# swapUniba/Deep_CBRS_Amar_Renaissance

Measured on AMD Instinct MI355X. Metric: (user,item) pairs scored/sec, ML-1M basic-gnn 2-layer, 1/2/4/8 MI355X, higher is better.
Workload: dtype f32; 1 GPU; ml1m(s=64) user-item graph: N=590592 nodes, nnz(A_hat)=55909934, 12089292 test pairs; econfigs/basic-gnn.yaml grid1 BasicGCN d=8 L=2 concat, dense [24,24], clf [48,48]; one propagation + per-entity towers + all pairs (shuffled order) per step (hoisted); scale=64, parallelism=single GPU (step replayed from a hipGraph)

## Files before the change

### deep_cbrs_amar_renaissance_amd/capi.py

```python
import ctypes
import os

import torch

_HERE = os.path.dirname(os.path.abspath(__file__))
LIB_PATH = os.path.join(_HERE, 'libamar_hip.so')

ACT_NONE, ACT_RELU, ACT_SIGMOID = 0, 1, 2
ACT_CODES = {None: ACT_NONE, 'linear': ACT_NONE, 'relu': ACT_RELU, 'sigmoid': ACT_SIGMOID}
AGG_SUM, AGG_MAX, AGG_MIN = 0, 1, 2
AGG_CODES = {'sum': AGG_SUM, 'max': AGG_MAX, 'min': AGG_MIN}
SPMM_BIAS, SPMM_RELU, SPMM_ACCUM, SPMM_ACCUM_DIV, SPMM_SCALE_NEXT, SPMM_SAGE_TAIL, SPMM_LT_NOPAIRS = 1, 2, 4, 8, 16, 32, 64

_P = ctypes.c_void_p
_I32, _I64, _U32, _F32 = ctypes.c_int32, ctypes.c_int64, ctypes.c_uint32, ctypes.c_float

SIGNATURES = {
    'amar_version': (ctypes.c_int, []),
    'amar_error_string': (ctypes.c_char_p, [ctypes.c_int]),
    'amar_last_hip_error': (ctypes.c_int, []),
    'amar_spmm_csr_f32': (ctypes.c_int, [_P, _P, _P, _P, _I64, _P, _I64, _I32, _I32, _U32, _P,
                                         _P, _I64, _P, _I64, _F32, _P]),
    'amar_spmm_sj_f32': (ctypes.c_int, [_P, _P, _P, _I32, _P, _I64, _P, _I64, _I32, _I32, _U32, _P,
                                        _P, _I64, _P, _I64, _F32, _P, _I32, _P, _I64, _P]),
    'amar_spmm_xs_f32': (ctypes.c_int, [_P, _P, _P, _P, _P, _I32, _P, _I64, _I32, _P, _P, _P, _I64, _I32, _I32, _U32, _P,
                                        _P, _I64, _P, _I64, _F32, _P, _I32, _P, _I64, _P]),
    'amar_gat_lt_f32': (ctypes.c_int, [_P, _P, _P, _P, _P, _P, _P, _I32, _I32, _I32, _I32, _P, _P, _P, _P, _I64, _I32, _P, _P, _P, _P, _P, _I64,
                                       _I32, _I32, _I32, _I32, _P]),
    'amar_gat_lt_rows_per_wave': (ctypes.c_int, [_I32]),
    'amar_colmax_f32': (ctypes.c_int, [_P, _I64, _P, _P]),
    'amar_spmm_lt_f32': (ctypes.c_int, [_P, _P, _P, _P, _P, _P, _P, _I32, _I32, _I32, _P, _P, _P, _I64, _I32, _P, _P, _I64, _I32, _I32, _U32, _P,
                                        _P, _I64, _P, _I64, _F32, _P, _I32, _P, _I64, _P]),
    'amar_gat_xs_f32': (ctypes.c_int, [_P, _P, _I32, _P, _I64, _I32, _P, _P, _P, _P, _P, _P, _I64, _I32, _I32, _I32, _I32, _P]),
    'amar_gcn_layer_f32': (ctypes.c_int, [_P, _P, _P, _P, _I64, _I32, _P, _P, _I64, _P, _I32, _P, _I64, _I32, _P]),
    'amar_rowwise_xw_f32': (ctypes.c_int, [_P, _I64, _I32, _P, _I32, _P, _I64, _P, _I64, _P, _P, _P, _P, _P, _I32, _P]),
    'amar_rowwise_xw_gather_f32': (ctypes.c_int, [_P, _I64, _I32, _P, _P, _I32, _P, _I64, _P, _I32, _P]),
    'amar_sage_layer_f32': (ctypes.c_int, [_P, _P, _P, _I64, _I32, _P, _P, _I32, _P, _I64, _I32, _I32, _P]),
    'amar_sage_tail_f32': (ctypes.c_int, [_P, _I64, _P, _I64, _I32, _P, _P, _I32, _P, _I64, _I64, _P]),
    'amar_sage_layer_agg_f32': (ctypes.c_int, [_P, _P, _P, _I64, _I32, _P, _P, _I32, _P, _I64, _I32, _I32, _I32, _P]),
    'amar_sage_aggregate_f32': (ctypes.c_int, [_P, _P, _P, _I64, _I32, _P, _I64, _P, _I64, _I32, _I32, _I32, _P]),
    'amar_sage_aggregate_bwd_f32': (ctypes.c_int, [_P, _P, _P, _I64, _P, _I64, _P, _I64, _P, _I64, _I32, _P, _P, _I64, _I32, _I32, _P]),
    'amar_gat_layer_f32': (ctypes.c_int, [_P, _P, _P, _I64, _I32, _P, _P, _P, _P, _I64, _I32, _I32, _P]),
    'amar_rowwise_xw_heads_f32': (ctypes.c_int, [_P, _I64, _I32, _P, _I32, _I32, _P, _I64, _P, _P, _P, _I32, _P]),
    'amar_gat_heads_f32': (ctypes.c_int, [_P, _P, _P, _I64, _I32, _I32, _P, _P, _P, _I64, _P, _I32, _I32, _I32, _P]),
    'amar_dense_f32': (ctypes.c_int, [_P, _I64, _P, _P, _P, _P, _I64, _I64, _I32, _I32, _I32, _P]),
    'amar_dense_split_bytes': (ctypes.c_int64, [_I32, _I32]),
    'amar_dense_split_pack_f32': (ctypes.c_int, [_P, _I32, _I32, _P]),
    'amar_dense_split_f32': (ctypes.c_int, [_P, _I64, _P, _P, _P, _P, _I64, _I64, _I32, _I32, _I32, _P]),
    'amar_chain_pack_floats': (ctypes.c_int64, [_P, _I32]),
    'amar_chain_pack_f32': (ctypes.c_int, [_P, _P, _P, _I32, _P]),
    'amar_chain_f32': (ctypes.c_int, [_P, _I64, _I32, _P, _I32, _P, _I64, _I32, _P, _I32, _I32, _I32, _P, _P, _P, _I32, _P, _I64, _I64, _P]),
    'amar_chain_indexed_f32': (ctypes.c_int, [_P, _I64, _I32, _P, _I32, _P, _I64, _I32, _P, _I32, _I32, _I32, _P, _P, _P, _I32, _P, _I64, _P, _I64, _P]),
    'amar_chain_segments_f32': (ctypes.c_int, [_P, _P, _P, _I32, _P, _I32, _P, _P, _P, _I32, _P, _I64, _I64, _P]),
    'amar_chain_route': (ctypes.c_int, [_P, _I64, _I32, _P, _I32, _P, _I64, _I32, _P, _I32, _I32, _I32, _P, _P, _P, _I32, _P, _I64, _P, _I64, _P]),
    'amar_chain_segments_route': (ctypes.c_int, [_P, _P, _P, _I32, _P, _I32, _P, _P, _P, _I32, _P, _I64, _I64, _P]),
    'amar_dual_chain_f32': (ctypes.c_int, [_P, _P, _P, _P, _P, _P, _P, _P, _I32, _I32, _I32, _P, _P, _P, _I32, _P, _P, _I64, _I64, _P]),
    'amar_dual_chain_indexed_f32': (ctypes.c_int, [_P, _P, _P, _P, _P, _P, _P, _P, _I32, _I32, _I32, _P, _P, _P, _I32, _P, _P, _I64, _P, _I64, _P]),
    'amar_copy_columns_f32': (ctypes.c_int, [_P, _I64, _P, _I32, _P, _I64, _I64, _I32, _P]),
    'amar_scatter_f32': (ctypes.c_int, [_P, _P, _P, _I64, _I64, _P, _I32, _P]),
    'amar_reduce_layers_f32': (ctypes.c_int, [_P, _I64, _I32, _I32, _P, _I64, _I64, _I32, _P]),
    'amar_reduce_layers_wsum_f32': (ctypes.c_int, [_P, _I64, _I32, _I32, _P, _P, _I64, _I64, _P]),
    'amar_reduce_layers_wsum_bwd_scratch': (ctypes.c_int64, []),
    'amar_reduce_layers_wsum_bwd_f32': (ctypes.c_int, [_P, _I64, _I32, _I32, _P, _P, _I64, _P, _I64, _P, _P, _I64, _P]),
    'amar_act_bwd_f32': (ctypes.c_int, [_P, _I64, _P, _I64, _P, _I64, _I64, _I32, _I32, _P]),
    'amar_wgrad_scratch_floats': (ctypes.c_int64, [_I64, _I32, _I32]),
    'amar_wgrad_f32': (ctypes.c_int, [_P, _I64, _P, _I64, _I64, _I32, _I32, _P, _P, _P, _P]),
    'amar_dense_stack_f32': (ctypes.c_int, [_P, _I64, _P, _P, _I64, _I32, _P, _P, _P, _P, _P, _P, _I64, _P]),
    'amar_dense_stack_pair_f32': (ctypes.c_int, [_P, _P, _P]),
    'amar_dense_stack_route': (ctypes.c_int, [_P, _I64, _P, _P, _I64, _I32, _P, _P, _P, _P, _P, _P, _I64, _P]),
    'amar_dense_stack_bwd_groups': (ctypes.c_int64, [_I64]),
    'amar_dense_stack_bwd_workspace_floats': (ctypes.c_int64, [_I64, _I32, _P]),
    'amar_dense_stack_bwd_pair_f32': (ctypes.c_int, [_P, _P, _P]),
    'amar_dense_stack_bwd_f32': (ctypes.c_int, [_P, _I64, _P, _I64, _I32, _P, _P, _P, _P, _P, _P, _I64, _P, _P, _P, _I32, _I64, _P]),
    'amar_dense_stack_bwd_route': (ctypes.c_int, [_P, _I64, _P, _I64, _I32, _P, _P, _P, _P, _P, _P, _I64, _P, _P, _P, _I32, _I64, _P]),
    'amar_dense_bwd_workspace_floats': (ctypes.c_int64, [_I64, _I32, _I32]),
    'amar_dense_bwd_groups': (ctypes.c_int64, [_I64]),
    'amar_dense_bwd_f32': (ctypes.c_int, [_P, _I64, _P, _I64, _P, _I64, _P, _I32, _P, _I64, _P, _P, _P, _I64, _P, _I64, _I32, _I32, _P]),
    'amar_dense_bwd_route': (ctypes.c_int, [_P, _I64, _P, _I64, _P, _I64, _P, _I32, _P, _I64, _P, _P, _P, _I64, _I64, _I32, _I32, _P]),
    'amar_bce_grad_f32': (ctypes.c_int, [_P, _I64, _P, _P, _P, _I64, _P]),
    'amar_wgrad_route': (ctypes.c_int, [_P, _I64, _P, _I64, _I64, _I32, _I32, _P, _P, _P]),
    'amar_scatter_add_rows_route': (ctypes.c_int, [_I64, _I32, _P]),
    'amar_scatter_add_rows_f32': (ctypes.c_int, [_P, _I64, _P, _I32, _P, _I64, _I64, _I32, _P]),
    'amar_add_inplace_f32': (ctypes.c_int, [_P, _I64, _P, _I64, _I64, _I32, _F32, _P]),
    'amar_row_affine_f32': (ctypes.c_int, [_P, _I64, _P, _I64, _P, _P, _I64, _I64, _I32, _P]),
    'amar_l2norm_fwd_f32': (ctypes.c_int, [_P, _I64, _P, _I64, _P, _P, _I64, _I64, _I32, _I32, _P]),
    'amar_l2norm_bwd_f32': (ctypes.c_int, [_P, _I64, _P, _I64, _P, _P, _I64, _I64, _I32, _I32, _P]),
    'amar_gat_bwd_f32': (ctypes.c_int, [_P, _P, _P, _I64, _I32, _P, _P, _P, _I64, _P, _I64, _P, _P, _P, _P, _P, _P, _P, _P, _I64,
                                        _I32, _I32, _P]),
    'amar_gat_bwd_directed_f32': (ctypes.c_int, [_P, _P, _P, _P, _P, _I64, _I32, _P, _P, _P, _I64, _P, _I64, _P, _P, _P, _P, _P, _P, _P, _P, _I64,
                                                 _I32, _I32, _P]),
    'amar_gat_heads_bwd_f32': (ctypes.c_int, [_P, _P, _P, _P, _P, _I64, _I32, _I32, _P, _P, _I64, _P, _I64, _P, _P, _P, _P, _P, _P, _P, _P, _I64,
                                              _I32, _I32, _I32, _P]),
    'amar_attention_mix_f32': (ctypes.c_int, [_P, _I64, _P, _I64, _P, _I64, _P, _I64, _P, _I64, _I64, _I32, _P]),
    'amar_attention_mix_bwd_f32': (ctypes.c_int, [_P, _I64, _P, _I64, _P, _I64, _P, _I64, _P, _I64, _P, _P, _P, _P, _I64, _I32, _P]),
    'amar_add3_act_f32': (ctypes.c_int, [_P, _I64, _P, _I64, _P, _I64, _P, _I64, _I64, _I32, _I32, _P]),
    'amar_locality_scale_f32': (ctypes.c_int, [_P, _I64, _P, _P, _I64, _I64, _I32, _P]),
    'amar_locality_scale_bwd_f32': (ctypes.c_int, [_P, _I64, _P, _I64, _P, _P, _I64, _P, _I64, _I32, _I32, _P]),
    'amar_transpose_f32': (ctypes.c_int, [_P, _I32, _I32, _P, _P]),
    'amar_adam_f32': (ctypes.c_int, [_P, _P, _P, _P, _I64, _F32, _F32, _F32, _F32, _F32, _P]),
    'amar_adam_advance_f32': (ctypes.c_int, [_P, _F32, _F32, _F32, _P]),
    'amar_adam_dev_f32': (ctypes.c_int, [_P, _P, _P, _P, _I64, _P, _F32, _F32, _F32, _F32, _P]),
    'amar_optim_state_arrays': (ctypes.c_int, [_I32, _I32, _F32]),
    'amar_optim_advance_f32': (ctypes.c_int, [_P, _I32, _I32, _P, _P]),
    'amar_optim_f32': (ctypes.c_int, [_I32, _I32, _P, _P, _P, _P, _P, _P, _I64, _P, _F32, _P]),
    'amar_optim_multi_f32': (ctypes.c_int, [_I32, _I32, _P, _P, _I32, _I64, _P, _F32, _P, _P]),
    'amar_grad_clip_workspace_floats': (ctypes.c_int64, [_I32, _I64]),
    'amar_grad_clip_f32': (ctypes.c_int, [_I32, _F32, _P, _I32, _I64, _P, _P, _F32, _P, _P]),
    'amar_bpr_grad_f32': (ctypes.c_int, [_P, _I64, _P, _P, _I64, _P]),
    'amar_bpr_sample_i32': (ctypes.c_int, [_P, _P, _P, _P, _I32, ctypes.c_uint64, _P, _I32, _I32, _P, _P, _P, _P]),
    'amar_loss_counters': (ctypes.c_int32, []),
    'amar_loss_grad_f32': (ctypes.c_int, [_I32, _P, _P, _I64, _P, _P, _P, _I64, _P, _P]),
    'amar_dropout_f32': (ctypes.c_int, [_P, _I64, _P, _I64, _I64, _I32, ctypes.c_uint64, _P, _U32, _U32, _F32, _P]),
    'amar_dropout_advance': (ctypes.c_int, [_P, _P]),
    'amar_gat_layer_dropout_f32': (ctypes.c_int, [_P, _P, _P, _I64, _I32, _P, _P, _P, _P, _I64, _I32, _I32,
                                                  ctypes.c_uint64, _P, _U32, _U32, _F32, _P]),
    'amar_gat_bwd_dropout_f32': (ctypes.c_int, [_P, _P, _P, _I64, _I32, _P, _P, _P, _I64, _P, _I64, _P, _P, _P, _P, _P, _P, _P, _P, _I64,
                                                _I32, _I32, ctypes.c_uint64, _P, _U32, _U32, _F32, _P]),
    'amar_gat_bwd_directed_dropout_f32': (ctypes.c_int, [_P, _P, _P, _P, _P, _I64, _I32, _P, _P, _P, _I64, _P, _I64, _P, _P, _P, _P, _P, _P, _P, _P,
                                                         _I64, _I32, _I32, ctypes.c_uint64, _P, _U32, _U32, _F32, _P]),
    'amar_csr_transpose_i32': (ctypes.c_int, [_P, _P, _I32, _I32, _I32, _P, _P, _P, _P, _P]),
    'amar_adam_multi_f32': (ctypes.c_int, [_P, _I32, _I64, _P, _F32, _F32, _F32, _F32, _P, _P]),
    'amar_sum_into_f32': (ctypes.c_int, [_P, _I64, _F32, _P, _P]),
    'amar_topk_segmented_f32': (ctypes.c_int, [_P, _P, _P, _I32, _I32, _P, _P, _P]),
    'amar_recommend_slices': (ctypes.c_int32, [_I64, _I32, _P, _I32, _I32]),
    'amar_recommend_f32': (ctypes.c_int, [_P, _I64, _I32, _P, _I64, _I32, _I32, _P, _P, _P, _I32, _I32, _P, _I64, _P, _P,
                                          _I32, _I32, _P, _P, _P, _P, _P]),
}

_lib = None


class AmarError(RuntimeError):
    pass


def load():
    global _lib
    if _lib is None:
        if not os.path.exists(LIB_PATH):
            raise AmarError(
                "{} is missing: build it with `python -c 'import __graft_entry__ as g; g.build()'` "
                "or `make -C deep_cbrs_amar_renaissance_amd/csrc`. The HIP path has no fallback.".format(LIB_PATH))
# ... 565 lines not shown

class ConcatTable:

    def __init__(self, tables):
        tables = list(tables)
        if not tables:
            raise ValueError("ConcatTable: at least one table expected")
        rows = int(tables[0].shape[0])
        if any(t.dim() != 2 or int(t.shape[0]) != rows or t.dtype != torch.float32 for t in tables):
            raise ValueError("ConcatTable: float32 [rows, w] tables with equal row counts expected")
        self.in_place = all(int(t.shape[1]) % 4 == 0 for t in tables)
        self.segments = tables
        self.shape = (rows, sum(int(t.shape[1]) for t in tables))
        self.device, self.dtype = tables[0].device, torch.float32

    def __getitem__(self, key):
        if not isinstance(key, slice) or key.step not in (None, 1):
            raise TypeError("ConcatTable supports contiguous row slices only")
        return ConcatTable([t[key] for t in self.segments])

    def materialize(self):
        out = torch.empty(self.shape, dtype=torch.float32, device=self.device)
        off = 0
        for t in self.segments:
            copy_columns(t, out[:, off:off + t.shape[1]])
            off += t.shape[1]
        return out


def _chain_segments_args(table, wpack, dims, acts, out, ids=None, base=0):
    P = out.shape[0]
    segs = table.segments
    if ids is not None and ids.numel() != P:
        raise ValueError("chain: ids must have one id per output row")
    if ids is None and table.shape[0] < P:
        raise ValueError("chain: input blocks have fewer rows than the output")
    n = len(segs)
    ptrs = (ctypes.c_void_p * n)(*[_ptr(t, torch.float32, 'segment') for t in segs])
    lds = (ctypes.c_int64 * n)(*[_ld(t, 'segment') for t in segs])
    ws = (ctypes.c_int32 * n)(*[int(t.shape[1]) for t in segs])
    dims_c = (ctypes.c_int32 * len(dims))(*dims)
    acts_c = (ctypes.c_int32 * len(acts))(*[ACT_CODES[a] for a in acts])
    return [ptrs, lds, ws, n, _ptr(ids, torch.int32, 'ids'), int(base), _ptr(wpack, torch.float32, 'wpack'), dims_c, acts_c, len(acts),
            _ptr(out, torch.float32, 'out'), _ld(out, 'out'), P]


def chain_segments(table, wpack, dims, acts, out, ids=None, base=0):
    code = load().amar_chain_segments_f32(*_chain_segments_args(table, wpack, dims, acts, out, ids=ids, base=base), _stream())
    if code == -2:
        return False
    _check(code, 'amar_chain_segments_f32')
    return True


def _chain_args(A, wpack, dims, acts, out, ids_a=None, base_a=0, B=None, ids_b=None, base_b=0, sum_inputs=False, in_act=None, out_index=None):
    P = out.shape[0]
    Da, Db = A.shape[1], (B.shape[1] if B is not None else 0)
    for ids, nm in ((ids_a, 'ids_a'), (ids_b, 'ids_b')):
        if ids is not None and ids.numel() != P:
            raise ValueError("chain: {} must have one id per output row".format(nm))
    if ids_a is None and A.shape[0] < P or (B is not None and ids_b is None and B.shape[0] < P):
        raise ValueError("chain: input blocks have fewer rows than the output")
    dims_c = (ctypes.c_int32 * len(dims))(*dims)
    acts_c = (ctypes.c_int32 * len(acts))(*[ACT_CODES[a] for a in acts])
    if out_index is not None and out_index.numel() != P:
        raise ValueError("chain: out_index must have one entry per output row")
    return [_ptr(A, torch.float32, 'A'), _ld(A, 'A'), Da, _ptr(ids_a, torch.int32, 'ids_a'), int(base_a),
            _ptr(B, torch.float32, 'B'), _ld(B, 'B') if B is not None else 0, Db, _ptr(ids_b, torch.int32, 'ids_b'), int(base_b),
            1 if sum_inputs else 0, ACT_CODES[in_act],
            _ptr(wpack, torch.float32, 'wpack'), dims_c, acts_c, len(acts),
            _ptr(out, torch.float32, 'out'), _ld(out, 'out'), _ptr(out_index, torch.int32, 'out_index'), P]


def chain(A, wpack, dims, acts, out, ids_a=None, base_a=0, B=None, ids_b=None, base_b=0, sum_inputs=False, in_act=None, out_index=None):
    if isinstance(A, ConcatTable):
        if A.in_place and B is None and not sum_inputs and out_index is None and chain_segments(A, wpack, dims, acts, out, ids=ids_a, base=base_a):
            return
        A = A.materialize()
    args = _chain_args(A, wpack, dims, acts, out, ids_a=ids_a, base_a=base_a, B=B, ids_b=ids_b, base_b=base_b, sum_inputs=sum_inputs,
                       in_act=in_act, out_index=out_index)
    _check(load().amar_chain_indexed_f32(*args, _stream()), 'amar_chain_indexed_f32' if out_index is not None else 'amar_chain_f32')


CHAIN_KERNEL_GENERIC, CHAIN_KERNEL_PIPE, CHAIN_KERNEL_ROWS = 0, 1, 2


class ChainRouteInfo(ctypes.Structure):
    _fields_ = [(name, ctypes.c_int32) for name in ('kernel', 'maxt', 'full', 'am', 'split', 'scatter', 'shape', 'lastlin', 'seg', 'has_dot',
                                                    'layers', 'threads')] + [('blocks', ctypes.c_int64), ('lds_bytes', ctypes.c_int64)]

    def as_dict(self):
        d = {name: int(getattr(self, name)) for name, _ in self._fields_}
        for name in ('full', 'split', 'scatter', 'lastlin', 'seg', 'has_dot'):
            d[name] = bool(d[name])
        return d


def chain_shape(*tiles):
    code = len(tiles) - 1
    for j, t in enumerate(tiles):
        code |= t << (3 * (j + 1))
    return code


def chain_route(A, wpack, dims, acts, out, ids_a=None, base_a=0, B=None, ids_b=None, base_b=0, sum_inputs=False, in_act=None, out_index=None):
    info = ChainRouteInfo()
    if isinstance(A, ConcatTable):
        if not (A.in_place and B is None and not sum_inputs and out_index is None):
            raise ValueError("chain_route: this ConcatTable call is assembled first; ask about the assembled table")
        args = _chain_segments_args(A, wpack, dims, acts, out, ids=ids_a, base=base_a)
        _check(load().amar_chain_segments_route(*args, ctypes.byref(info)), 'amar_chain_segments_route')
        return info.as_dict()
    args = _chain_args(A, wpack, dims, acts, out, ids_a=ids_a, base_a=base_a, B=B, ids_b=ids_b, base_b=base_b, sum_inputs=sum_inputs,
                       in_act=in_act, out_index=out_index)
    _check(load().amar_chain_route(*args, ctypes.byref(info)), 'amar_chain_route')
    return info.as_dict()


def dual_chain_supported(D, n_branch_dims_equal, trunk_dims):
    return (D % 16 == 0 and D <= 64 and n_branch_dims_equal and len(trunk_dims) >= 3 and trunk_dims[0] == 2 * D
            and trunk_dims[-1] == 1 and len(set(trunk_dims[1:-1])) == 1 and trunk_dims[1] <= 64 and trunk_dims[1] % 4 == 0)


def dual_chain(tables_a, tables_b, ids_a, ids_b, bases_a, bases_b, D, in_act, branch_acts, trunk_dims, trunk_acts, wpack, out,
               out_index=None):
    P = out.shape[0]
    arr = lambda vals, ctype: (ctype * 2)(*vals)
    A = arr([_ptr(t, torch.float32, 'A') for t in tables_a], ctypes.c_void_p)
    B = arr([_ptr(t, torch.float32, 'B') for t in tables_b], ctypes.c_void_p)
    IA = arr([_ptr(t, torch.int32, 'ida') for t in ids_a], ctypes.c_void_p)
    IB = arr([_ptr(t, torch.int32, 'idb') for t in ids_b], ctypes.c_void_p)
    for ids in list(ids_a) + list(ids_b):
        if ids is not None and ids.numel() != P:
            raise ValueError("dual_chain: one id per output row expected")
    lda = arr([_ld(t, 'A') for t in tables_a], ctypes.c_int64)
    ldb = arr([_ld(t, 'B') for t in tables_b], ctypes.c_int64)
    ba, bb = arr([int(b) for b in bases_a], ctypes.c_int32), arr([int(b) for b in bases_b], ctypes.c_int32)
    bacts = (ctypes.c_int32 * max(1, len(branch_acts)))(*[ACT_CODES[a] for a in branch_acts])
    tdims = (ctypes.c_int32 * len(trunk_dims))(*trunk_dims)
    tacts = (ctypes.c_int32 * len(trunk_acts))(*[ACT_CODES[a] for a in trunk_acts])
    if out_index is not None and out_index.numel() != P:
        raise ValueError("dual_chain: out_index must have one entry per output row")
    code = load().amar_dual_chain_indexed_f32(A, lda, IA, ba, B, ldb, IB, bb, D, ACT_CODES[in_act], len(branch_acts), bacts,
                                              tdims, tacts, len(trunk_acts), _ptr(wpack, torch.float32, 'wpack'),
                                              _ptr(out, torch.float32, 'out'), _ld(out, 'out'), _ptr(out_index, torch.int32, 'out_index'),
                                              P, _stream())
    _check(code, 'amar_dual_chain_f32' if out_index is None else 'amar_dual_chain_indexed_f32')


def scatter(src, index, dst, window_off=None, n_windows=1):
    n = int(index.numel())
    if src.numel() < n or (window_off is not None and window_off.numel() != n_windows + 1):
        raise ValueError("scatter: one source value per index and n_windows + 1 window offsets expected")
    if n == 0:
        return
    _check(load().amar_scatter_f32(_ptr(src, torch.float32, 'src'), _ptr(index, torch.int32, 'index'), _ptr(dst, torch.float32, 'dst'),
                                   _ld(dst, 'dst') if dst.dim() == 2 else 1, n, _ptr(window_off, torch.int32, 'window_off'),
                                   int(n_windows), _stream()), 'amar_scatter_f32')


def copy_columns(src, dst, ids=None, base=0):
    n = ids.numel() if ids is not None else src.shape[0]
    if src.shape[1] != dst.shape[1] or dst.shape[0] != n:
        raise ValueError("copy_columns: shapes differ")
    code = load().amar_copy_columns_f32(_ptr(src, torch.float32, 'src'), _ld(src, 'src'),
                                        _ptr(ids, torch.int32, 'ids'), int(base),
                                        _ptr(dst, torch.float32, 'dst'), _ld(dst, 'dst'),
                                        n, src.shape[1], _stream())
    _check(code, 'amar_copy_columns_f32')


def reduce_layers(cat, n_layers, width, out, mean=False):
    if cat.shape[1] != n_layers * width or tuple(out.shape) != (cat.shape[0], width):
        raise ValueError("reduce_layers: cat [n, n_layers*width], out [n, width] expected")
    code = load().amar_reduce_layers_f32(_ptr(cat, torch.float32, 'cat'), _ld(cat, 'cat'), n_layers, width,
                                         _ptr(out, torch.float32, 'out'), _ld(out, 'out'), cat.shape[0],
                                         1 if mean else 0, _stream())
    _check(code, 'amar_reduce_layers_f32')


def reduce_layers_wsum(cat, n_layers, width, w, out):
    if cat.shape[1] != n_layers * width or tuple(out.shape) != (cat.shape[0], width) or w.numel() != n_layers or not w.is_contiguous():
        raise ValueError("reduce_layers_wsum: cat [n, n_layers*width], w [n_layers], out [n, width] expected")
    code = load().amar_reduce_layers_wsum_f32(_ptr(cat, torch.float32, 'cat'), _ld(cat, 'cat'), n_layers, width, _ptr(w, torch.float32, 'w'),
                                              _ptr(out, torch.float32, 'out'), _ld(out, 'out'), cat.shape[0], _stream())
    _check(code, 'amar_reduce_layers_wsum_f32')


def reduce_layers_wsum_bwd(cat, n_layers, width, w, d_out, d_cat, dw):
    n = cat.shape[0]
    if (cat.shape[1] != n_layers * width or tuple(d_cat.shape) != tuple(cat.shape) or tuple(d_out.shape) != (n, width)
            or w.numel() != n_layers or dw.numel() != n_layers or not w.is_contiguous() or not dw.is_contiguous()):
        raise ValueError("reduce_layers_wsum_bwd: cat / d_cat [n, n_layers*width], d_out [n, width], w / dw [n_layers] expected")
    scratch = torch.empty(int(load().amar_reduce_layers_wsum_bwd_scratch()), dtype=torch.float32, device=cat.device)
    code = load().amar_reduce_layers_wsum_bwd_f32(_ptr(cat, torch.float32, 'cat'), _ld(cat, 'cat'), n_layers, width, _ptr(w, torch.float32, 'w'),
                                                  _ptr(d_out, torch.float32, 'd_out'), _ld(d_out, 'd_out'),
                                                  _ptr(d_cat, torch.float32, 'd_cat'), _ld(d_cat, 'd_cat'), _ptr(dw, torch.float32, 'dw'),
                                                  _ptr(scratch, torch.float32, 'scratch'), n, _stream())
    _check(code, 'amar_reduce_layers_wsum_bwd_f32')


def adam_advance(state, learning_rate, beta_1, beta_2):
    if state.numel() != 2 or not state.is_contiguous():
        raise ValueError("adam_advance: state must be 2 contiguous floats (t, lr_t)")
    _check(load().amar_adam_advance_f32(_ptr(state, torch.float32, 'state'), float(learning_rate), float(beta_1), float(beta_2),
                                        _stream()), 'amar_adam_advance_f32')


def adam_dev(w, g, m, v, state, beta_1, beta_2, epsilon, l2=0.0):
    if not (w.is_contiguous() and g.is_contiguous() and m.is_contiguous() and v.is_contiguous()) or \
            not (w.numel() == g.numel() == m.numel() == v.numel()):
        raise ValueError("adam_dev: contiguous tensors of equal size expected")
    code = load().amar_adam_dev_f32(_ptr(w, torch.float32, 'w'), _ptr(g, torch.float32, 'g'), _ptr(m, torch.float32, 'm'),
                                    _ptr(v, torch.float32, 'v'), w.numel(), _ptr(state, torch.float32, 'state'), float(beta_1),
                                    float(beta_2), float(epsilon), float(l2), _stream())
    _check(code, 'amar_adam_dev_f32')


class DeferredGradient:

    def __init__(self, partials, groups, shape):
        self.partials, self.groups, self.shape = partials, int(groups), tuple(shape)

    def materialize(self):
        parts = self.partials.view(self.groups, -1)
        total = torch.zeros_like(parts[0])
        for g in range(self.groups):
            total += parts[g]
        return total.view(self.shape)


def flat_gradient(g):
    return g if isinstance(g, DeferredGradient) else g.contiguous().view(-1)


class AdamSlot(ctypes.Structure):
    _fields_ = [('w', ctypes.c_void_p), ('g', ctypes.c_void_p), ('m', ctypes.c_void_p), ('v', ctypes.c_void_p),
# ... 819 lines not shown
```

### deep_cbrs_amar_renaissance_amd/csrc/amar_chain.hip

```cpp
#include "amar_common.h"
#include <stdlib.h>
#include <string.h>

namespace {

typedef float f32x4 __attribute__((ext_vector_type(4)));

constexpr int CHAIN_MAX_LAYERS = 8;
constexpr int CHAIN_MAX_SEG = 8;

struct ChainArgs {
    const float *A; int64_t lda; int Da; const int32_t *ids_a; int base_a;
    int n_seg; const float *seg[CHAIN_MAX_SEG]; int64_t seg_ld[CHAIN_MAX_SEG]; int seg_off[CHAIN_MAX_SEG + 1];
    const float *B; int64_t ldb; int Db; const int32_t *ids_b; int base_b;
    const float *wpack; int wpack_floats;
    int sum_inputs, in_act;
    int n_layers;
    int kt[CHAIN_MAX_LAYERS], nt[CHAIN_MAX_LAYERS], act[CHAIN_MAX_LAYERS];
    int w_off[CHAIN_MAX_LAYERS], b_off[CHAIN_MAX_LAYERS];
    int has_dot, dot_off, dot_bias_off, dot_act, dot_kt;
    int n_out;
    float *out; int64_t ldo; int64_t P;
    const int32_t *out_index;
};

__device__ __forceinline__ int64_t chain_out_row(const ChainArgs &a, int64_t p) { return a.out_index ? (int64_t)a.out_index[p] : p; }

__device__ __forceinline__ float chain_act(float v, int act) {
    if (act == AMAR_ACT_RELU) return fmaxf(v, 0.f);
    if (act == AMAR_ACT_SIGMOID) return 1.f / (1.f + expf(-v));
    return v;
}

template <bool RELU>
__device__ __forceinline__ float chain_act_t(float v, int act) { return RELU ? fmaxf(v, 0.f) : chain_act(v, act); }

template <int MAXT, int PT, bool FULL, int AM>
__global__ __launch_bounds__(256) void chain_kernel(const ChainArgs a) {
    constexpr bool RELU = AM != 0;
    extern __shared__ __attribute__((aligned(16))) float w_lds[];
    for (int i = threadIdx.x * 4; i < a.wpack_floats; i += blockDim.x * 4)
        *reinterpret_cast<float4 *>(&w_lds[i]) = *reinterpret_cast<const float4 *>(a.wpack + i);
    __syncthreads();

    const int lane = threadIdx.x & 63, g = lane >> 4, col = lane & 15;
    const int64_t pairs_per_wave = 16 * PT;
    const int64_t wave0 = (int64_t)blockIdx.x * 4 + (threadIdx.x >> 6);
    const int64_t stride = (int64_t)gridDim.x * 4 * pairs_per_wave;

    for (int64_t base = wave0 * pairs_per_wave; base < a.P; base += stride) {
        f32x4 x[MAXT][PT];
#pragma unroll
        for (int pt = 0; pt < PT; ++pt) {
            const int64_t p = base + 16 * pt + col;
            const bool ok = p < a.P;
            const int64_t ra = ok ? (a.ids_a ? (int64_t)a.ids_a[p] - a.base_a : p) : 0;
            const int64_t rb = (ok && a.Db) ? (a.ids_b ? (int64_t)a.ids_b[p] - a.base_b : p) : 0;
#pragma unroll
            for (int t = 0; t < MAXT; ++t) {
                const int f = 16 * t + 4 * g;
                f32x4 v = {0.f, 0.f, 0.f, 0.f};
                if ((FULL || t < a.kt[0]) && ok) {
                    if (a.sum_inputs) {
                        if (f < a.Da) {
                            const f32x4 va = *reinterpret_cast<const f32x4 *>(a.A + ra * a.lda + f);
                            const f32x4 vb = *reinterpret_cast<const f32x4 *>(a.B + rb * a.ldb + f);
                            v = va + vb;
#pragma unroll
                            for (int r = 0; r < 4; ++r) v[r] = chain_act_t<RELU>(v[r], a.in_act);
                        }
                    } else if (f < a.Da) v = *reinterpret_cast<const f32x4 *>(a.A + ra * a.lda + f);
                    else if (f < a.Da + a.Db) v = *reinterpret_cast<const f32x4 *>(a.B + rb * a.ldb + (f - a.Da));
                }
                x[t][pt] = v;
            }
        }
        for (int l = 0; l < a.n_layers; ++l) {
            const int KT = FULL ? MAXT : a.kt[l], NT = FULL ? MAXT : a.nt[l];
            const float *wl = w_lds + a.w_off[l];
            const float *bl = w_lds + a.b_off[l];
            f32x4 y[MAXT][PT];
#pragma unroll
            for (int m = 0; m < MAXT; ++m) {
                if (FULL || m < NT) {
                    const f32x4 b4 = *reinterpret_cast<const f32x4 *>(bl + 16 * m + 4 * g);
#pragma unroll
                    for (int pt = 0; pt < PT; ++pt) y[m][pt] = b4;
#pragma unroll
                    for (int t = 0; t < MAXT; ++t) {
                        if (FULL || t < KT) {
                            const f32x4 w4 = *reinterpret_cast<const f32x4 *>(wl + ((m * KT + t) * 64 + lane) * 4);
#pragma unroll
                            for (int r = 0; r < 4; ++r)
#pragma unroll
                                for (int pt = 0; pt < PT; ++pt)
                                    y[m][pt] = __builtin_amdgcn_mfma_f32_16x16x4f32(w4[r], x[t][pt][r], y[m][pt], 0, 0, 0);
                        }
                    }
                }
            }
            const int act = a.act[l];
            if (AM == 2 && l == a.n_layers - 1) {
#pragma unroll
                for (int m = 0; m < MAXT; ++m)
#pragma unroll
                    for (int pt = 0; pt < PT; ++pt) {
                        const f32x4 zero = {0.f, 0.f, 0.f, 0.f};
                        x[m][pt] = (FULL || m < NT) ? y[m][pt] : zero;
                    }
            } else {
#pragma unroll
                for (int m = 0; m < MAXT; ++m)
#pragma unroll
                    for (int pt = 0; pt < PT; ++pt) {
                        f32x4 v = {0.f, 0.f, 0.f, 0.f};
                        if (FULL || m < NT) {
                            v = y[m][pt];
#pragma unroll
                            for (int r = 0; r < 4; ++r) v[r] = chain_act_t<RELU>(v[r], act);
                        }
                        x[m][pt] = v;
                    }
            }
        }
        if (a.has_dot) {
            const float *wd = w_lds + a.dot_off;
            const float bd = w_lds[a.dot_bias_off];
#pragma unroll
            for (int pt = 0; pt < PT; ++pt) {
                float s = 0.f;
#pragma unroll
                for (int t = 0; t < MAXT; ++t) {
                    if (FULL || t < a.dot_kt) {
                        const f32x4 w4 = *reinterpret_cast<const f32x4 *>(wd + 16 * t + 4 * g);
#pragma unroll
                        for (int r = 0; r < 4; ++r) s = fmaf(x[t][pt][r], w4[r], s);
                    }
                }
                s += __shfl_xor(s, 16, 64);
                s += __shfl_xor(s, 32, 64);
                const int64_t p = base + 16 * pt + col;
                if (g == 0 && p < a.P) a.out[chain_out_row(a, p) * a.ldo] = chain_act(s + bd, a.dot_act);
            }
        } else {
#pragma unroll
            for (int pt = 0; pt < PT; ++pt) {
                const int64_t p = base + 16 * pt + col;
#pragma unroll
                for (int m = 0; m < MAXT; ++m) {
                    const int f = 16 * m + 4 * g;
                    if (p < a.P && f < a.n_out) *reinterpret_cast<f32x4 *>(a.out + chain_out_row(a, p) * a.ldo + f) = x[m][pt];
                }
            }
        }
    }
}

__device__ __forceinline__ float relu_bits(float v) { return __int_as_float(max(__float_as_int(v), 0)); }

constexpr int chain_shape(int nl, int t0, int t1, int t2 = 0, int t3 = 0) { return nl | t0 << 3 | t1 << 6 | t2 << 9 | t3 << 12; }
constexpr int shape_nl(int s) { return s & 7; }
constexpr int shape_t(int s, int j) { return (s >> (3 * (j + 1))) & 7; }
constexpr int shape_maxt(int s) {
    int m = 0;
    for (int j = 0; j <= shape_nl(s); ++j) m = shape_t(s, j) > m ? shape_t(s, j) : m;
    return m;
}

template <int SHAPE, int PT, bool LASTLIN, bool SEG>
__global__ __launch_bounds__(256) void chain_rows_kernel(const ChainArgs a) {
    constexpr int NL = shape_nl(SHAPE), T0 = shape_t(SHAPE, 0), TN = shape_t(SHAPE, NL), MAXT = shape_maxt(SHAPE);
    extern __shared__ __attribute__((aligned(16))) float w_lds[];
    for (int i = threadIdx.x * 4; i < a.wpack_floats; i += blockDim.x * 4)
        *reinterpret_cast<float4 *>(&w_lds[i]) = *reinterpret_cast<const float4 *>(a.wpack + i);
    __syncthreads();

    const int lane = threadIdx.x & 63, g = lane >> 4, col = lane & 15;
    constexpr uint32_t rows_per_wave = 16 * PT;
    const uint32_t stride = gridDim.x * 4 * rows_per_wave;
    const uint32_t P = (uint32_t)a.P, last = P - 1;
    const uint32_t lda = (uint32_t)a.lda * 4u;
    const int f_last = 16 * (T0 - 1) + 4 * g;
    const bool tail_ok = f_last < a.Da;
    const char *Ag = reinterpret_cast<const char *>(a.A) + 16 * g;
    const int tail_off = tail_ok ? 64 * (T0 - 1) : -16 * g;
    const char *seg_base[SEG ? T0 : 1];
    uint32_t seg_ldb[SEG ? T0 : 1];
    if constexpr (SEG) {
#pragma unroll
        for (int t = 0; t < T0; ++t) {
            const int f = 16 * t + 4 * g;
            int sidx = 0;
            for (int j = 1; j < a.n_seg; ++j) sidx = (f < a.Da && f >= a.seg_off[j]) ? j : sidx;
            seg_base[t] = reinterpret_cast<const char *>(a.seg[sidx] + (f < a.Da ? f - a.seg_off[sidx] : 0));
            seg_ldb[t] = (uint32_t)a.seg_ld[sidx] * 4u;
        }
    }

    f32x4 xin[MAXT][PT];
    auto gather = [&](uint32_t b) {
#pragma unroll
        for (int pt = 0; pt < PT; ++pt) {
            const uint32_t p = min(b + 16 * pt + col, last);
            const uint32_t row = a.ids_a ? (uint32_t)(a.ids_a[p] - a.base_a) : p;
            const char *pa = Ag + (uint64_t)row * lda;
#pragma unroll
            for (int t = 0; t < T0; ++t) {
                if constexpr (SEG) xin[t][pt] = *reinterpret_cast<const f32x4 *>(seg_base[t] + (uint64_t)row * seg_ldb[t]);
                else xin[t][pt] = *reinterpret_cast<const f32x4 *>(pa + (t == T0 - 1 ? tail_off : 64 * t));
            }
        }
    };

    uint32_t base = (blockIdx.x * 4 + (threadIdx.x >> 6)) * rows_per_wave;
    if (base >= P) return;
    gather(base);
    for (; base < P; base += stride) {
        f32x4 x[MAXT][PT];
#pragma unroll
        for (int l = 0; l < NL; ++l) {
            const int KT = shape_t(SHAPE, l), NT = shape_t(SHAPE, l + 1);
            const float *wl = w_lds + a.w_off[l];
            const float *bl = w_lds + a.b_off[l];
            f32x4 y[MAXT][PT];
#pragma unroll
            for (int m = 0; m < MAXT; ++m) {
                if (m < NT) {
                    const f32x4 b4 = *reinterpret_cast<const f32x4 *>(bl + 16 * m + 4 * g);
#pragma unroll
                    for (int pt = 0; pt < PT; ++pt) y[m][pt] = b4;
#pragma unroll
                    for (int t = 0; t < MAXT; ++t) {
                        if (t < KT) {
                            const f32x4 w4 = *reinterpret_cast<const f32x4 *>(wl + ((m * KT + t) * 64 + lane) * 4);
#pragma unroll
                            for (int r = 0; r < 4; ++r)
#pragma unroll
                                for (int pt = 0; pt < PT; ++pt) {
                                    float xv = l == 0 ? xin[t][pt][r] : x[t][pt][r];
                                    if (l == 0 && t == T0 - 1) xv = tail_ok ? xv : 0.f;
                                    y[m][pt] = __builtin_amdgcn_mfma_f32_16x16x4f32(w4[r], xv, y[m][pt], 0, 0, 0);
                                }
                        }
                    }
                }
            }
            if (l == 0) gather(base + stride);
#pragma unroll
            for (int m = 0; m < MAXT; ++m)
#pragma unroll
                for (int pt = 0; pt < PT; ++pt)
                    if (m < NT) {
#pragma unroll
                        for (int r = 0; r < 4; ++r) x[m][pt][r] = (LASTLIN && l == NL - 1) ? y[m][pt][r] : relu_bits(y[m][pt][r]);
                    }
        }
#pragma unroll
        for (int pt = 0; pt < PT; ++pt) {
            const uint32_t p = base + 16 * pt + col;
            float *po = a.out + (int64_t)p * a.ldo + 4 * g;
#pragma unroll
            for (int m = 0; m < TN; ++m)
                if (p < P && 16 * m + 4 * g < a.n_out) *reinterpret_cast<f32x4 *>(po + 16 * m) = x[m][pt];
        }
    }
}


typedef uint32_t u32x4 __attribute__((ext_vector_type(4)));
typedef __bf16 bf16x8 __attribute__((ext_vector_type(8)));

struct Split3 { uint32_t h, m, l; };
typedef float f32x2 __attribute__((ext_vector_type(2)));
typedef uint32_t u32x2 __attribute__((ext_vector_type(2)));
__device__ __forceinline__ Split3 split_pair(float a, float b) {
    const f32x2 x = {a, b};
    const u32x2 xb = __builtin_bit_cast(u32x2, x);
    Split3 q;
    q.h = __builtin_amdgcn_perm(xb[1], xb[0], 0x07060302u);
    const f32x2 r1 = x - __builtin_bit_cast(f32x2, xb & 0xffff0000u);
    const u32x2 r1b = __builtin_bit_cast(u32x2, r1);
    q.m = __builtin_amdgcn_perm(r1b[1], r1b[0], 0x07060302u);
    const f32x2 r2 = r1 - __builtin_bit_cast(f32x2, r1b & 0xffff0000u);
    const u32x2 r2b = __builtin_bit_cast(u32x2, r2);
    q.l = __builtin_amdgcn_perm(r2b[1], r2b[0], 0x07060302u);
    return q;
}

struct Split3x4 { u32x4 h, m, l; };
__device__ __forceinline__ Split3x4 split_tiles(const f32x4 &t0, const f32x4 &t1) {
    const Split3 q0 = split_pair(t0[0], t0[1]), q1 = split_pair(t0[2], t0[3]), q2 = split_pair(t1[0], t1[1]), q3 = split_pair(t1[2], t1[3]);
    Split3x4 o;
    o.h[0] = q0.h; o.h[1] = q1.h; o.h[2] = q2.h; o.h[3] = q3.h;
    o.m[0] = q0.m; o.m[1] = q1.m; o.m[2] = q2.m; o.m[3] = q3.m;
    o.l[0] = q0.l; o.l[1] = q1.l; o.l[2] = q2.l; o.l[3] = q3.l;
    return o;
}
__device__ __forceinline__ f32x4 split_mfma(const u32x4 *w, const Split3x4 &x, f32x4 acc) {
    const bf16x8 wh = __builtin_bit_cast(bf16x8, w[0]), wm = __builtin_bit_cast(bf16x8, w[64]), wl = __builtin_bit_cast(bf16x8, w[128]);
    const bf16x8 xh = __builtin_bit_cast(bf16x8, x.h), xm = __builtin_bit_cast(bf16x8, x.m), xl = __builtin_bit_cast(bf16x8, x.l);
    acc = __builtin_amdgcn_mfma_f32_16x16x32_bf16(wl, xh, acc, 0, 0, 0);
    acc = __builtin_amdgcn_mfma_f32_16x16x32_bf16(wh, xl, acc, 0, 0, 0);
    acc = __builtin_amdgcn_mfma_f32_16x16x32_bf16(wm, xm, acc, 0, 0, 0);
    acc = __builtin_amdgcn_mfma_f32_16x16x32_bf16(wm, xh, acc, 0, 0, 0);
    acc = __builtin_amdgcn_mfma_f32_16x16x32_bf16(wh, xm, acc, 0, 0, 0);
    acc = __builtin_amdgcn_mfma_f32_16x16x32_bf16(wh, xh, acc, 0, 0, 0);
    return acc;
}

template <int MAXT, int PT, bool SCATTER, bool SPLIT>
__global__ __launch_bounds__(256) void chain_pipe_kernel(const ChainArgs a) {
    extern __shared__ __attribute__((aligned(16))) float w_lds[];
    for (int i = threadIdx.x * 4; i < a.wpack_floats; i += blockDim.x * 4)
        *reinterpret_cast<float4 *>(&w_lds[i]) = *reinterpret_cast<const float4 *>(a.wpack + i);
    __syncthreads();

    const int lane = threadIdx.x & 63, g = lane >> 4, col = lane & 15;
    constexpr int KS = (MAXT + 1) / 2;
    constexpr bool BIASK = SPLIT && (MAXT & 1);
    u32x4 *frag = reinterpret_cast<u32x4 *>(w_lds + ((a.wpack_floats + 3) & ~3));
    if (SPLIT) {
        for (int idx = threadIdx.x >> 6; idx < a.n_layers * MAXT * KS; idx += 4) {
            const int l = idx / (MAXT * KS), m = (idx % (MAXT * KS)) / KS, sk = idx % KS;
            const float *wl = w_lds + a.w_off[l];
            const f32x4 wa = *reinterpret_cast<const f32x4 *>(wl + ((m * MAXT + 2 * sk) * 64 + lane) * 4);
            f32x4 wb = {0.f, 0.f, 0.f, 0.f};
            if (2 * sk + 1 < MAXT) wb = *reinterpret_cast<const f32x4 *>(wl + ((m * MAXT + 2 * sk + 1) * 64 + lane) * 4);
            else if (BIASK && g == 0) wb[0] = w_lds[a.b_off[l] + 16 * m + col];
            u32x4 *dst = frag + idx * 3 * 64 + lane;
            const Split3 q0 = split_pair(wa[0], wa[1]), q1 = split_pair(wa[2], wa[3]), q2 = split_pair(wb[0], wb[1]), q3 = split_pair(wb[2], wb[3]);
            u32x4 h, mm, lo;
            h[0] = q0.h; h[1] = q1.h; h[2] = q2.h; h[3] = q3.h;
            mm[0] = q0.m; mm[1] = q1.m; mm[2] = q2.m; mm[3] = q3.m;
            lo[0] = q0.l; lo[1] = q1.l; lo[2] = q2.l; lo[3] = q3.l;
            dst[0] = h; dst[64] = mm; dst[128] = lo;
        }
        __syncthreads();
    }
    constexpr uint32_t pairs_per_wave = 16 * PT;
    const uint32_t wave0 = blockIdx.x * 4 + (threadIdx.x >> 6);
    const uint32_t stride = gridDim.x * 4 * pairs_per_wave;
    const uint32_t P = (uint32_t)a.P, last = P - 1;
    const char *Ag = reinterpret_cast<const char *>(a.A + 4 * g), *Bg = reinterpret_cast<const char *>(a.B + 4 * g);
// ... 707 lines not shown
            a.has_dot = 1; a.dot_off = off; a.dot_kt = tiles16(K); a.dot_act = act;
            off += 16 * tiles16(K);
            a.dot_bias_off = off;
            off += 4;
        } else {
            maxw = N > maxw ? N : maxw;
            a.kt[a.n_layers] = tiles16(K); a.nt[a.n_layers] = tiles16(N); a.act[a.n_layers] = act;
            a.w_off[a.n_layers] = off;
            off += tiles16(N) * tiles16(K) * 256;
            a.b_off[a.n_layers] = off;
            off += 16 * tiles16(N);
            a.n_layers++;
            a.n_out = N;
        }
    }
    a.wpack_floats = off;
    if (a.n_layers < 1) return AMAR_EINVAL;
    if (!a.has_dot && ((ldo & 3) || ldo < a.n_out || (a.n_out & 3) || !amar_aligned16(out))) return AMAR_EINVAL;
    if (a.has_dot && ldo < 1) return AMAR_EINVAL;
    if (maxw > 128 || (size_t)off * sizeof(float) > 150 * 1024) return AMAR_EUNSUPPORTED;
    const size_t lds_bytes = (size_t)off * sizeof(float);
    const int maxt = maxw <= 48 ? 3 : (maxw <= 64 ? 4 : 8);
    bool full = (dims[0] + 15) / 16 == maxt && (!a.has_dot || a.dot_kt == maxt);
    for (int l = 0; l < a.n_layers; ++l) full = full && a.kt[l] == maxt && a.nt[l] == maxt;
    bool relu = !a.sum_inputs || a.in_act == AMAR_ACT_RELU, relu_but_last = relu && !a.has_dot;
    for (int l = 0; l < a.n_layers; ++l) {
        relu = relu && a.act[l] == AMAR_ACT_RELU;
        relu_but_last = relu_but_last && a.act[l] == (l == a.n_layers - 1 ? AMAR_ACT_NONE : AMAR_ACT_RELU);
    }
    const int am = relu ? 1 : (relu_but_last ? 2 : 0);
    r.maxt = maxt; r.full = full; r.am = am; r.has_dot = a.has_dot; r.layers = a.n_layers; r.threads = 256;
    r.lds_bytes = (int64_t)lds_bytes;
    const int64_t tiles = (P + 4 * 16 * 2 - 1) / (4 * 16 * 2);
    const bool a_dot_ok = !a.has_dot || a.dot_kt == maxt;
    const bool small_tables = lda < (1ll << 30) && ldb < (1ll << 30) && P < (1ll << 30) - (4ll << 20);
    if (relu && a.sum_inputs && a.in_act == AMAR_ACT_RELU && full && a_dot_ok && a.ids_a && a.ids_b && a.Da == 16 * maxt &&
        a.Db == a.Da && maxt <= 4 && lds_bytes <= 64 * 1024 && small_tables && (a.has_dot || !a.out_index)) {
        static const bool f32_only = getenv("AMAR_PAIR_MFMA") && !strcmp(getenv("AMAR_PAIR_MFMA"), "f32");
        const size_t split_bytes = (((size_t)off + 3) & ~(size_t)3) * sizeof(float) + (size_t)a.n_layers * maxt * ((maxt + 1) / 2) * 3 * 1024;
        r.kernel = AMAR_CHAIN_KERNEL_PIPE;
        r.split = !f32_only && split_bytes <= 64 * 1024;
        r.scatter = a.out_index != nullptr;
        r.blocks = tiles > 1536 ? 1536 : tiles;
        if (r.split) r.lds_bytes = (int64_t)split_bytes;
        return AMAR_OK;
    }
    if ((am == 1 || am == 2) && !a.sum_inputs && a.Db == 0 && !a.has_dot && !a.out_index && a.n_layers <= 3 &&
        maxt <= 4 && lds_bytes <= 64 * 1024 && lda < (1ll << 30) && P < (1ll << 30) - (4ll << 20)) {
        const int shape = chain_shape(a.n_layers, a.kt[0], a.nt[0], a.n_layers > 1 ? a.nt[1] : 0, a.n_layers > 2 ? a.nt[2] : 0);
        if (chain_rows_shape_known(shape)) {
            r.kernel = AMAR_CHAIN_KERNEL_ROWS;
            r.shape = shape; r.lastlin = am == 2; r.seg = n_seg > 0;
            r.blocks = tiles > 1024 ? 1024 : tiles;
            return AMAR_OK;
        }
    }
    if (n_seg > 0 && P > 0) return AMAR_EUNSUPPORTED;
    r.kernel = AMAR_CHAIN_KERNEL_GENERIC;
    r.blocks = tiles > 4096 ? 4096 : tiles;
    return AMAR_OK;
}

int amar_chain_route(const float *A, int64_t lda, int32_t Da, const int32_t *ids_a, int32_t base_a,
                     const float *B, int64_t ldb, int32_t Db, const int32_t *ids_b, int32_t base_b,
                     int32_t sum_inputs, int32_t in_act,
                     const float *wpack, const int32_t *dims, const int32_t *acts, int32_t n_layers,
                     float *out, int64_t ldo, const int32_t *out_index, int64_t P, amar_chain_route_info *info) {
    if (!info) return AMAR_EINVAL;
    ChainArgs a;
    return chain_route(A, lda, Da, ids_a, base_a, B, ldb, Db, ids_b, base_b, sum_inputs, in_act, wpack, dims, acts, n_layers, out, ldo, out_index, P,
                       0, nullptr, nullptr, nullptr, a, *info);
}

int amar_chain_segments_route(const float *const *seg, const int64_t *seg_ld, const int32_t *seg_width, int32_t n_seg,
                              const int32_t *ids, int32_t base,
                              const float *wpack, const int32_t *dims, const int32_t *acts, int32_t n_layers,
                              float *out, int64_t ldo, int64_t P, amar_chain_route_info *info) {
    if (!info) return AMAR_EINVAL;
    int64_t da = 0;
    if (const int rc = chain_segments_check(seg, seg_ld, seg_width, n_seg, &da)) return rc;
    ChainArgs a;
    return chain_route(seg[0], seg_ld[0], (int32_t)da, ids, base, nullptr, 0, 0, nullptr, 0, 0, AMAR_ACT_NONE, wpack, dims, acts, n_layers, out, ldo,
                       nullptr, P, n_seg, seg, seg_ld, seg_width, a, *info);
}

static int chain_run(const float *A, int64_t lda, int32_t Da, const int32_t *ids_a, int32_t base_a,
                     const float *B, int64_t ldb, int32_t Db, const int32_t *ids_b, int32_t base_b,
                     int32_t sum_inputs, int32_t in_act,
                     const float *wpack, const int32_t *dims, const int32_t *acts, int32_t n_layers,
                     float *out, int64_t ldo, const int32_t *out_index, int64_t P, amar_stream_t stream,
                     int32_t n_seg, const float *const *seg, const int64_t *seg_ld, const int32_t *seg_width) {
    ChainArgs a;
    amar_chain_route_info r;
    if (const int rc = chain_route(A, lda, Da, ids_a, base_a, B, ldb, Db, ids_b, base_b, sum_inputs, in_act, wpack, dims, acts, n_layers, out, ldo,
                                   out_index, P, n_seg, seg, seg_ld, seg_width, a, r))
        return rc;
    if (r.blocks == 0) return AMAR_OK;
    hipStream_t st = static_cast<hipStream_t>(stream);
    const dim3 grid((unsigned)r.blocks), block((unsigned)r.threads);
    const size_t lds = (size_t)r.lds_bytes;
    if (r.kernel == AMAR_CHAIN_KERNEL_PIPE) {
#define AMAR_PIPE_LAUNCH(MT, SC)                                                                                          \
        do {                                                                                                              \
            if (r.split) hipLaunchKernelGGL((chain_pipe_kernel<MT, 2, SC, true>), grid, block, lds, st, a);               \
            else hipLaunchKernelGGL((chain_pipe_kernel<MT, 2, SC, false>), grid, block, lds, st, a);                      \
        } while (0)
        if (r.scatter) {
            if (r.maxt == 3) AMAR_PIPE_LAUNCH(3, true); else AMAR_PIPE_LAUNCH(4, true);
        } else {
            if (r.maxt == 3) AMAR_PIPE_LAUNCH(3, false); else AMAR_PIPE_LAUNCH(4, false);
        }
#undef AMAR_PIPE_LAUNCH
        return amar_check_launch();
    }
    if (r.kernel == AMAR_CHAIN_KERNEL_ROWS) {
#define AMAR_ROWS_CASE(NLL, A0, A1, A2, A3)                                                                                      \
        case chain_shape(NLL, A0, A1, A2, A3):                                                                                   \
            if (r.seg) {                                                                                                         \
                if (r.lastlin) hipLaunchKernelGGL((chain_rows_kernel<chain_shape(NLL, A0, A1, A2, A3), 2, true, true>), grid, block, lds, st, a);   \
                else hipLaunchKernelGGL((chain_rows_kernel<chain_shape(NLL, A0, A1, A2, A3), 2, false, true>), grid, block, lds, st, a);            \
            } else if (r.lastlin) hipLaunchKernelGGL((chain_rows_kernel<chain_shape(NLL, A0, A1, A2, A3), 2, true, false>), grid, block, lds, st, a);   \
            else hipLaunchKernelGGL((chain_rows_kernel<chain_shape(NLL, A0, A1, A2, A3), 2, false, false>), grid, block, lds, st, a);            \
            break;
        switch (r.shape) {
        AMAR_ROWS_SHAPES(AMAR_ROWS_CASE)
        default: return AMAR_EUNSUPPORTED;
        }
#undef AMAR_ROWS_CASE
        return amar_check_launch();
    }
#define AMAR_CHAIN_LAUNCH(MT)                                                                                           \
    do {                                                                                                                \
        auto kern = r.full ? (r.am == 1 ? chain_kernel<MT, 2, true, 1> : r.am == 2 ? chain_kernel<MT, 2, true, 2>       \
                                                                                 : chain_kernel<MT, 2, true, 0>)        \
                           : (r.am == 1 ? chain_kernel<MT, 2, false, 1> : r.am == 2 ? chain_kernel<MT, 2, false, 2>     \
                                                                                  : chain_kernel<MT, 2, false, 0>);     \
        if (lds > 64 * 1024 &&                                                                                          \
            hipFuncSetAttribute(reinterpret_cast<const void *>(kern), hipFuncAttributeMaxDynamicSharedMemorySize,       \
                                (int)lds) != hipSuccess)                                                                \
            return AMAR_ELAUNCH;                                                                                        \
        hipLaunchKernelGGL(kern, grid, block, lds, st, a);                                                              \
    } while (0)
    if (r.maxt == 3) AMAR_CHAIN_LAUNCH(3); else if (r.maxt == 4) AMAR_CHAIN_LAUNCH(4); else AMAR_CHAIN_LAUNCH(8);
#undef AMAR_CHAIN_LAUNCH
    return amar_check_launch();
}

int amar_dual_chain_f32(const float *const *A, const int64_t *lda, const int32_t *const *ida, const int32_t *base_a,
                        const float *const *B, const int64_t *ldb, const int32_t *const *idb, const int32_t *base_b,
                        int32_t D, int32_t in_act, int32_t n_branch, const int32_t *branch_acts,
                        const int32_t *trunk_dims, const int32_t *trunk_acts, int32_t n_trunk,
                        const float *wpack, float *out, int64_t ldo, int64_t P, amar_stream_t stream) {
    return amar_dual_chain_indexed_f32(A, lda, ida, base_a, B, ldb, idb, base_b, D, in_act, n_branch, branch_acts, trunk_dims, trunk_acts,
                                       n_trunk, wpack, out, ldo, nullptr, P, stream);
}

int amar_dual_chain_indexed_f32(const float *const *A, const int64_t *lda, const int32_t *const *ida, const int32_t *base_a,
                                const float *const *B, const int64_t *ldb, const int32_t *const *idb, const int32_t *base_b,
                                int32_t D, int32_t in_act, int32_t n_branch, const int32_t *branch_acts,
                                const int32_t *trunk_dims, const int32_t *trunk_acts, int32_t n_trunk,
                                const float *wpack, float *out, int64_t ldo, const int32_t *out_index, int64_t P, amar_stream_t stream) {
    if (P < 0 || !A || !B || !lda || !ldb || !ida || !idb || !base_a || !base_b || !wpack || !out || !trunk_dims || !trunk_acts)
        return AMAR_EINVAL;
    if (D < 4 || (D & 3) || n_branch < 0 || n_branch > CHAIN_MAX_LAYERS || (n_branch && !branch_acts)) return AMAR_EINVAL;
    if (n_trunk < 2 || n_trunk > CHAIN_MAX_LAYERS || trunk_dims[0] != 2 * D || trunk_dims[n_trunk] != 1 || ldo < 1) return AMAR_EINVAL;
    if (D > 64) return AMAR_EUNSUPPORTED;
    DualArgs a{};
    for (int b = 0; b < 2; ++b) {
        if (!A[b] || !B[b] || lda[b] < D || ldb[b] < D || (lda[b] & 3) || (ldb[b] & 3) || !amar_aligned16(A[b]) || !amar_aligned16(B[b]))
            return AMAR_EINVAL;
        a.A[b] = A[b]; a.lda[b] = lda[b]; a.ida[b] = ida[b]; a.base_a[b] = base_a[b];
        a.B[b] = B[b]; a.ldb[b] = ldb[b]; a.idb[b] = idb[b]; a.base_b[b] = base_b[b];
    }
    a.D = D; a.tb = tiles16(D); a.in_act = in_act; a.n_branch = n_branch;
    int off = 0;
    for (int b = 0; b < 2; ++b)
        for (int l = 0; l < n_branch; ++l) {
            a.bw_off[b][l] = off; off += a.tb * a.tb * 256;
            a.bb_off[b][l] = off; off += 16 * a.tb;
            a.b_act[l] = branch_acts[l];
        }
    const int W = trunk_dims[1];
    if (W < 4 || (W & 3) || W > 64) return AMAR_EUNSUPPORTED;
    a.tt = tiles16(W); a.n_trunk = n_trunk - 1;
    for (int l = 0; l < n_trunk - 1; ++l) {
        if (trunk_dims[l + 1] != W) return AMAR_EUNSUPPORTED;
        const int KT = l == 0 ? 2 * a.tb : a.tt;
        if (l == 0 && (D & 15)) return AMAR_EUNSUPPORTED;
        a.tw_off[l] = off; off += a.tt * KT * 256;
        a.tbias_off[l] = off; off += 16 * a.tt;
        a.t_act[l] = trunk_acts[l];
    }
    a.dot_off = off; off += 16 * a.tt;
    a.dot_bias_off = off; off += 4;
    a.dot_act = trunk_acts[n_trunk - 1];
    a.wpack = wpack; a.wpack_floats = off; a.out = out; a.ldo = ldo; a.P = P; a.out_index = out_index;
    if ((size_t)off * sizeof(float) > 150 * 1024) return AMAR_EUNSUPPORTED;
    if (P == 0) return AMAR_OK;
    const size_t lds_bytes = (size_t)off * sizeof(float);
    constexpr int PT = 1;
    constexpr int THREADS = 1024;
    int64_t blocks = (P + (THREADS / 64) * 16 * PT - 1) / ((THREADS / 64) * 16 * PT);
    if (blocks > 1024) blocks = 1024;
    bool full = D == 64 && W == 64 && in_act == AMAR_ACT_RELU && n_branch >= 1 && ida[0] && ida[1] && idb[0] && idb[1];
    for (int b = 0; b < 2; ++b) full = full && lda[b] < (1ll << 32) && ldb[b] < (1ll << 32);
    for (int l = 0; l < n_branch; ++l) full = full && branch_acts[l] == AMAR_ACT_RELU;
    for (int l = 0; l < n_trunk - 1; ++l) full = full && trunk_acts[l] == AMAR_ACT_RELU;
    static const bool f32_only = getenv("AMAR_PAIR_MFMA") && !strcmp(getenv("AMAR_PAIR_MFMA"), "f32");
    if (full && !f32_only && n_branch >= 1) {
        int nf = 0, tl = 0;
        for (int b = 0; b < 2; ++b)
            for (int l = 0; l < n_branch; ++l) { a.bw_frag[b][l] = nf; nf += 4 * 2; a.bb_tail[b][l] = tl; tl += 64; }
        for (int l = 0; l < a.n_trunk; ++l) { a.tw_frag[l] = nf; nf += 4 * (l == 0 ? 4 : 2); a.tb_tail[l] = tl; tl += 64; }
        a.dot_tail = tl; tl += 64; a.dot_bias_tail = tl; tl += 4;
        a.n_frag = nf; a.tail_floats = tl;
        const size_t bytes = (size_t)nf * 3 * 1024 + (size_t)tl * sizeof(float);
        if (bytes <= 160 * 1024) {
            static bool lds_ok[AMAR_MAX_DEVICES];
            if (bytes > 64 * 1024)
                if (const int rc = amar_allow_lds(reinterpret_cast<const void *>(dual_chain_split_kernel<1, 768>), 160 * 1024, lds_ok)) return rc;
            int64_t blocks3 = (P + 12 * 16 - 1) / (12 * 16);
            if (blocks3 > 1024) blocks3 = 1024;
            hipLaunchKernelGGL((dual_chain_split_kernel<1, 768>), dim3((unsigned)blocks3), dim3(768), bytes, static_cast<hipStream_t>(stream), a);
            return amar_check_launch();
        }
    }
    auto kern = full ? dual_chain_full_kernel : dual_chain_kernel<PT>;
    if (lds_bytes > 64 * 1024 &&
// ... 8 lines not shown
```

### deep_cbrs_amar_renaissance_amd/csrc/amar_layout.hip

```cpp
#include "amar_common.h"

namespace {

__global__ __launch_bounds__(256) void copy_columns_kernel(const float *__restrict__ src, int64_t lds,
                                                           const int32_t *__restrict__ ids, int base,
                                                           float *__restrict__ dst, int64_t ldd, int64_t n_rows,
                                                           int width) {
    const int64_t total = n_rows * width;
    for (int64_t i = (int64_t)blockIdx.x * blockDim.x + threadIdx.x; i < total; i += (int64_t)gridDim.x * blockDim.x) {
        const int64_t r = i / width;
        const int c = (int)(i - r * width);
        const int64_t sr = ids ? (int64_t)ids[r] - base : r;
        dst[r * ldd + c] = src[sr * lds + c];
    }
}

__global__ __launch_bounds__(256) void copy_columns_vec_kernel(const float *__restrict__ src, int64_t lds,
                                                               const int32_t *__restrict__ ids, int base,
                                                               float *__restrict__ dst, int64_t ldd, int64_t n_rows,
                                                               int quads) {
    const int64_t total = n_rows * quads;
    for (int64_t i = (int64_t)blockIdx.x * blockDim.x + threadIdx.x; i < total; i += (int64_t)gridDim.x * blockDim.x) {
        const int64_t r = i / quads;
        const int q = (int)(i - r * quads);
// ... 13 lines not shown
        for (int l = 1; l < n_layers; ++l) s += cat[r * ld + (int64_t)l * width + c];
        out[r * ldo + c] = div != 0.f ? s / div : s;
    }
}

constexpr int WSUM_MAX_LAYERS = 8, WSUM_BWD_BLOCKS = 512;
__global__ __launch_bounds__(256) void reduce_layers_wsum_kernel(const float *__restrict__ cat, int64_t ld, int n_layers, int width,
                                                                 const float *__restrict__ w, float *__restrict__ out, int64_t ldo,
                                                                 int64_t n_rows) {
    float ww[WSUM_MAX_LAYERS];
    for (int l = 0; l < n_layers; ++l) ww[l] = __fmul_rn(w[l], w[l]);
    const int64_t total = n_rows * width;
    for (int64_t i = (int64_t)blockIdx.x * blockDim.x + threadIdx.x; i < total; i += (int64_t)gridDim.x * blockDim.x) {
        const int64_t r = i / width;
        const int c = (int)(i - r * width);
        float s = __fmul_rn(ww[0], cat[r * ld + c]);
        for (int l = 1; l < n_layers; ++l) s = __fadd_rn(s, __fmul_rn(ww[l], cat[r * ld + (int64_t)l * width + c]));
        out[r * ldo + c] = s;
    }
}

__global__ __launch_bounds__(256) void reduce_layers_wsum_bwd_kernel(const float *__restrict__ cat, int64_t ld, int n_layers, int width,
                                                                     const float *__restrict__ w, const float *__restrict__ d_out, int64_t ldd,
                                                                     float *__restrict__ d_cat, int64_t ldc, int64_t n_rows,
                                                                     float *__restrict__ partials) {
    __shared__ float red[4][WSUM_MAX_LAYERS];
    float ww[WSUM_MAX_LAYERS], acc[WSUM_MAX_LAYERS];
    for (int l = 0; l < WSUM_MAX_LAYERS; ++l) { ww[l] = l < n_layers ? w[l] * w[l] : 0.f; acc[l] = 0.f; }
    const int64_t total = n_rows * width;
    for (int64_t i = (int64_t)blockIdx.x * blockDim.x + threadIdx.x; i < total; i += (int64_t)gridDim.x * blockDim.x) {
        const int64_t r = i / width;
        const int c = (int)(i - r * width);
        const float g = d_out[r * ldd + c];
#pragma unroll
        for (int l = 0; l < WSUM_MAX_LAYERS; ++l)
            if (l < n_layers) {
                acc[l] = fmaf(g, cat[r * ld + (int64_t)l * width + c], acc[l]);
                d_cat[r * ldc + (int64_t)l * width + c] = ww[l] * g;
            }
    }
#pragma unroll
    for (int l = 0; l < WSUM_MAX_LAYERS; ++l) {
        float v = acc[l];
        for (int off = 32; off > 0; off >>= 1) v += __shfl_xor(v, off, 64);
        if ((threadIdx.x & 63) == 0) red[threadIdx.x >> 6][l] = v;
    }
    __syncthreads();
    if (threadIdx.x < WSUM_MAX_LAYERS)
        partials[(int64_t)blockIdx.x * WSUM_MAX_LAYERS + threadIdx.x] =
            ((red[0][threadIdx.x] + red[1][threadIdx.x]) + red[2][threadIdx.x]) + red[3][threadIdx.x];
}

__global__ __launch_bounds__(64) void reduce_layers_wsum_dw_kernel(const float *__restrict__ partials, int n_blocks, int n_layers,
                                                                   const float *__restrict__ w, float *__restrict__ dw) {
    const int l = blockIdx.x;
    float v = 0.f;
    for (int b = threadIdx.x; b < n_blocks; b += 64) v += partials[(int64_t)b * WSUM_MAX_LAYERS + l];
    for (int off = 32; off > 0; off >>= 1) v += __shfl_xor(v, off, 64);
    if (threadIdx.x == 0 && l < n_layers) dw[l] = 2.f * w[l] * v;
}

unsigned grid_for(int64_t total) {
    int64_t b = (total + 255) / 256;
    return (unsigned)(b > 4096 ? 4096 : (b < 1 ? 1 : b));
}

__global__ __launch_bounds__(256) void scatter_windows_kernel(const float *__restrict__ src, const int32_t *__restrict__ index,
                                                              float *__restrict__ dst, int64_t ldd, int64_t n,
                                                              const int32_t *__restrict__ window_off, int n_windows, int per_xcd) {
    const int x = blockIdx.x & 7, j = blockIdx.x >> 3;
    for (int w = x; w < n_windows; w += 8) {
        const int64_t lo = window_off ? window_off[w] : n * w / n_windows, hi = window_off ? window_off[w + 1] : n * (w + 1) / n_windows;
        const int64_t step = (int64_t)per_xcd * 256;
        int64_t t = lo + (int64_t)j * 256 + threadIdx.x;
        for (; t + 3 * step < hi; t += 4 * step) {
            const int32_t i0 = index[t], i1 = index[t + step], i2 = index[t + 2 * step], i3 = index[t + 3 * step];
            const float v0 = src[t], v1 = src[t + step], v2 = src[t + 2 * step], v3 = src[t + 3 * step];
            dst[(int64_t)i0 * ldd] = v0; dst[(int64_t)i1 * ldd] = v1; dst[(int64_t)i2 * ldd] = v2; dst[(int64_t)i3 * ldd] = v3;
        }
        for (; t < hi; t += step) dst[(int64_t)index[t] * ldd] = src[t];
    }
}

}

extern "C" {

int amar_copy_columns_f32(const float *src, int64_t lds, const int32_t *ids, int32_t base,
                          float *dst, int64_t ldd, int64_t n_rows, int32_t width, amar_stream_t stream) {
    if (n_rows < 0 || width < 1 || !src || !dst || lds < width || ldd < width) return AMAR_EINVAL;
    if (n_rows == 0) return AMAR_OK;
    if ((width & 3) == 0 && (lds & 3) == 0 && (ldd & 3) == 0 && amar_aligned16(src) && amar_aligned16(dst))
        hipLaunchKernelGGL(copy_columns_vec_kernel, dim3(grid_for(n_rows * (width / 4))), dim3(256), 0,
                           static_cast<hipStream_t>(stream), src, lds, ids, base, dst, ldd, n_rows, width / 4);
    else
        hipLaunchKernelGGL(copy_columns_kernel, dim3(grid_for(n_rows * width)), dim3(256), 0,
                           static_cast<hipStream_t>(stream), src, lds, ids, base, dst, ldd, n_rows, width);
    return amar_check_launch();
}

int amar_reduce_layers_f32(const float *cat, int64_t ld, int32_t n_layers, int32_t width, float *out, int64_t ldo,
                           int64_t n_rows, int32_t mean, amar_stream_t stream) {
    if (n_rows < 0 || n_layers < 1 || width < 1 || !cat || !out || ld < (int64_t)n_layers * width || ldo < width)
        return AMAR_EINVAL;
    if (n_rows == 0) return AMAR_OK;
    hipLaunchKernelGGL(reduce_layers_kernel, dim3(grid_for(n_rows * width)), dim3(256), 0,
                       static_cast<hipStream_t>(stream), cat, ld, n_layers, width, out, ldo, n_rows,
                       mean ? (float)n_layers : 0.f);
    return amar_check_launch();
}

int amar_reduce_layers_wsum_f32(const float *cat, int64_t ld, int32_t n_layers, int32_t width, const float *w, float *out, int64_t ldo,
                                int64_t n_rows, amar_stream_t stream) {
    if (n_rows < 0 || n_layers < 1 || width < 1 || !cat || !w || !out || ld < (int64_t)n_layers * width || ldo < width)
        return AMAR_EINVAL;
    if (n_layers > WSUM_MAX_LAYERS) return AMAR_EUNSUPPORTED;
    if (n_rows == 0) return AMAR_OK;
    hipLaunchKernelGGL(reduce_layers_wsum_kernel, dim3(grid_for(n_rows * width)), dim3(256), 0,
                       static_cast<hipStream_t>(stream), cat, ld, n_layers, width, w, out, ldo, n_rows);
    return amar_check_launch();
}

int64_t amar_reduce_layers_wsum_bwd_scratch(void) { return (int64_t)WSUM_BWD_BLOCKS * WSUM_MAX_LAYERS; }

int amar_reduce_layers_wsum_bwd_f32(const float *cat, int64_t ld, int32_t n_layers, int32_t width, const float *w,
                                    const float *d_out, int64_t ldd, float *d_cat, int64_t ld_dcat, float *dw, float *scratch,
                                    int64_t n_rows, amar_stream_t stream) {
    if (n_rows < 0 || n_layers < 1 || width < 1 || !cat || !w || !d_out || !d_cat || !dw || !scratch ||
        ld < (int64_t)n_layers * width || ld_dcat < (int64_t)n_layers * width || ldd < width)
        return AMAR_EINVAL;
    if (n_layers > WSUM_MAX_LAYERS) return AMAR_EUNSUPPORTED;
    hipStream_t st = static_cast<hipStream_t>(stream);
    int64_t blocks = (n_rows * width + 255) / 256;
    if (blocks > WSUM_BWD_BLOCKS) blocks = WSUM_BWD_BLOCKS;
    if (blocks < 1) blocks = 1;
    hipLaunchKernelGGL(reduce_layers_wsum_bwd_kernel, dim3((unsigned)blocks), dim3(256), 0, st, cat, ld, n_layers, width, w, d_out, ldd,
                       d_cat, ld_dcat, n_rows, scratch);
    hipLaunchKernelGGL(reduce_layers_wsum_dw_kernel, dim3((unsigned)n_layers), dim3(64), 0, st, scratch, (int)blocks, n_layers, w, dw);
    return amar_check_launch();
}

int amar_scatter_f32(const float *src, const int32_t *index, float *dst, int64_t ldd, int64_t n, const int32_t *window_off,
                     int32_t n_windows, amar_stream_t stream) {
    if (n < 0 || !src || !index || !dst || ldd < 1 || n_windows < 1 || n >= (1ll << 31)) return AMAR_EINVAL;
    if (n == 0) return AMAR_OK;
    constexpr int per_xcd = 32;
    hipLaunchKernelGGL(scatter_windows_kernel, dim3(8 * per_xcd), dim3(256), 0, static_cast<hipStream_t>(stream), src, index, dst, ldd, n,
                       window_off, n_windows, per_xcd);
    return amar_check_launch();
}
}
```

### deep_cbrs_amar_renaissance_amd/csrc/amar_propagate.hip

```cpp
#include "amar_common.h"
#include "amar_philox.h"
#include <stdlib.h>

namespace {

constexpr int WAVES_PER_BLOCK = 4;

template <int LPN, bool HAS_VALS>
__device__ __forceinline__ float4 row_gather_sum(const int32_t *__restrict__ colidx, const float *__restrict__ vals,
                                                 const float *__restrict__ X, int64_t ldx, int beg, int end,
                                                 int slot, int q) {
    constexpr int NS = AMAR_WAVE / LPN;
    float4 acc = f4_zero();
    int p = beg + slot;
    for (; p + NS < end; p += 2 * NS) {
        const int c0 = colidx[p], c1 = colidx[p + NS];
        const float v0 = HAS_VALS ? vals[p] : 1.f, v1 = HAS_VALS ? vals[p + NS] : 1.f;
        const float4 x0 = *reinterpret_cast<const float4 *>(X + (int64_t)c0 * ldx + 4 * q);
        const float4 x1 = *reinterpret_cast<const float4 *>(X + (int64_t)c1 * ldx + 4 * q);
        acc = f4_fma(v0, x0, acc);
        acc = f4_fma(v1, x1, acc);
    }
    if (p < end) {
        const int c0 = colidx[p];
// ... 868 lines not shown
#undef AMAR_LT_LAUNCH_P
    return amar_check_launch();
}

template <int F>
int launch_gat_lt(const LtArgs &a, int n_tiles, int off32, hipStream_t st) {
    constexpr int RW = lt_gat_rw(F);
    const size_t lds = (size_t)LT_WAVES * RW * (F + 2) * 4 + (size_t)LT_WAVES * LT_CHUNK * 4 + 32;
    static_assert((size_t)LT_WAVES * RW * (F + 2) * 4 + (size_t)LT_WAVES * LT_CHUNK * 4 + 32 <= (160u << 10), "one workgroup's LDS");
    const dim3 grid((unsigned)n_tiles), block(LT_WAVES * AMAR_WAVE);
#define AMAR_GAT_LT_LAUNCH(OFF)                                                                                          \
    do {                                                                                                                 \
        auto kern = spmm_lt_kernel<F, OFF, false, 4, 1, 0, true>;                                                        \
        static bool allowed[AMAR_MAX_DEVICES] = {};                                                                      \
        if (const int rc = amar_allow_lds(reinterpret_cast<const void *>(kern), lds, allowed)) return rc;               \
        hipLaunchKernelGGL(kern, grid, block, lds, st, a);                                                               \
    } while (0)
    if (off32 == 2) AMAR_GAT_LT_LAUNCH(2); else if (off32 == 1) AMAR_GAT_LT_LAUNCH(1); else AMAR_GAT_LT_LAUNCH(0);
#undef AMAR_GAT_LT_LAUNCH
    return amar_check_launch();
}

__global__ __launch_bounds__(256) void colmax_kernel(const float *__restrict__ x, int64_t n, float *out) {
    float m = -INFINITY;
    for (int64_t i = (int64_t)blockIdx.x * 256 + threadIdx.x; i < n; i += (int64_t)gridDim.x * 256) m = fmaxf(m, x[i]);
    m = wave_max_all(m);
    __shared__ float part[4];
    if ((threadIdx.x & 63) == 0) part[threadIdx.x >> 6] = m;
    __syncthreads();
    if (threadIdx.x == 0) {
        m = fmaxf(fmaxf(part[0], part[1]), fmaxf(part[2], part[3]));
        if (!(__builtin_bit_cast(unsigned, m) >> 31)) atomicMax(reinterpret_cast<int *>(out), __builtin_bit_cast(int, m));
        else atomicMin(reinterpret_cast<unsigned *>(out), __builtin_bit_cast(unsigned, m));
    }
}

bool ld_ok(int64_t ld, int F) { return ld >= F && (ld & 3) == 0; }

bool native_width(int F) { return F == 4 || F == 8 || F == 16 || F == 32 || F == 64; }
int chunk_width(int remaining) { return remaining >= 64 ? 64 : remaining >= 32 ? 32 : remaining >= 16 ? 16 : remaining >= 8 ? 8 : 4; }
const float *at(const float *p, int o) { return p ? p + o : nullptr; }
float *at(float *p, int o) { return p ? p + o : nullptr; }

struct XwArgs {
    const float *X; int64_t ldx; int F; const float *W; int C;
    float *H; int64_t ldh; float *copy_to; int64_t ld_copy;
    const float *a_self; const float *a_neigh; float *s_self; float *s_neigh;
    int n_rows;
    const float *row_scale;
    const int32_t *row_ids;
};

__global__ __launch_bounds__(256) void rowwise_xw_kernel(const XwArgs a, int CP) {
    extern __shared__ float w_lds[];
    for (int i = threadIdx.x; i < a.F * a.C; i += blockDim.x) w_lds[i] = a.W[i];
    __syncthreads();
    const int rows_per_block = blockDim.x / CP;
    const int c = threadIdx.x % CP, rslot = threadIdx.x / CP;
    for (int64_t row = (int64_t)blockIdx.x * rows_per_block + rslot; row < a.n_rows;
         row += (int64_t)gridDim.x * rows_per_block) {
        const int64_t src = a.row_ids ? (int64_t)a.row_ids[row] : row;
        const float *x = a.X + (src < 0 ? 0 : src) * a.ldx;
        float h = 0.f;
        if (c < a.C) {
            for (int k = 0; k < a.F; ++k) h = fmaf(x[k], w_lds[k * a.C + c], h);
            if (src < 0) h = 0.f;
            a.H[row * a.ldh + c] = a.row_scale ? h * a.row_scale[row] : h;
        }
        if (a.copy_to) for (int k = c; k < a.F; k += CP) a.copy_to[row * a.ld_copy + k] = x[k];
        if (a.s_self) {
            float ps = c < a.C ? h * a.a_self[c] : 0.f, pn = c < a.C ? h * a.a_neigh[c] : 0.f;
            for (int off = CP / 2; off >= 1; off >>= 1) { ps += __shfl_xor(ps, off, 64); pn += __shfl_xor(pn, off, 64); }
            if (c == 0) { a.s_self[row] = ps; a.s_neigh[row] = pn; }
        }
    }
}

template <int F>
__global__ __launch_bounds__(256) void rowwise_xw_vec_kernel(const XwArgs a) {
    __shared__ __attribute__((aligned(16))) float w_lds[F * F + 2 * F];
    for (int i = threadIdx.x; i < F * F; i += 256) w_lds[i] = a.W[i];
    if (a.s_self) for (int i = threadIdx.x; i < F; i += 256) { w_lds[F * F + i] = a.a_self[i]; w_lds[F * F + F + i] = a.a_neigh[i]; }
    __syncthreads();
    constexpr int R = F == 8 ? 2 : 1;
    for (int64_t row0 = (int64_t)blockIdx.x * 256 * R + threadIdx.x; row0 < a.n_rows; row0 += (int64_t)gridDim.x * 256 * R) {
        float x[R][F], sc[R];
        bool pad[R];
#pragma unroll
        for (int j = 0; j < R; ++j) {
            const int64_t row = row0 + 256 * j < a.n_rows ? row0 + 256 * j : row0;
            const int64_t src = a.row_ids ? (int64_t)a.row_ids[row] : row;
            pad[j] = src < 0;
            const int64_t xrow = pad[j] ? 0 : src;
#pragma unroll
            for (int q = 0; q < F / 4; ++q) {
                const float4 v = *reinterpret_cast<const float4 *>(a.X + xrow * a.ldx + 4 * q);
                x[j][4 * q] = v.x; x[j][4 * q + 1] = v.y; x[j][4 * q + 2] = v.z; x[j][4 * q + 3] = v.w;
            }
            sc[j] = pad[j] ? 0.f : (a.row_scale ? a.row_scale[row] : 1.f);
        }
#pragma unroll
        for (int j = 0; j < R; ++j) {
            const int64_t row = row0 + 256 * j;
            if (row >= a.n_rows) break;
            float h[F];
            if (a.copy_to) {
#pragma unroll
                for (int q = 0; q < F / 4; ++q)
                    *reinterpret_cast<float4 *>(a.copy_to + row * a.ld_copy + 4 * q) = make_float4(x[j][4 * q], x[j][4 * q + 1], x[j][4 * q + 2], x[j][4 * q + 3]);
            }
#pragma unroll
            for (int c = 0; c < F; ++c) h[c] = 0.f;
#pragma unroll
            for (int k = 0; k < F; ++k)
#pragma unroll
                for (int c4 = 0; c4 < F; c4 += 4) {
                    float4 w;
                    if (F == 8) {
                        const __attribute__((address_space(4))) float *wc = (const __attribute__((address_space(4))) float *)a.W;
                        w = make_float4(wc[k * F + c4], wc[k * F + c4 + 1], wc[k * F + c4 + 2], wc[k * F + c4 + 3]);
                    } else w = *reinterpret_cast<const float4 *>(&w_lds[k * F + c4]);
                    h[c4] = fmaf(x[j][k], w.x, h[c4]); h[c4 + 1] = fmaf(x[j][k], w.y, h[c4 + 1]);
                    h[c4 + 2] = fmaf(x[j][k], w.z, h[c4 + 2]); h[c4 + 3] = fmaf(x[j][k], w.w, h[c4 + 3]);
                }
#pragma unroll
            for (int q = 0; q < F / 4; ++q)
                *reinterpret_cast<float4 *>(a.H + row * a.ldh + 4 * q) = (a.row_scale || a.row_ids)
                    ? make_float4(h[4 * q] * sc[j], h[4 * q + 1] * sc[j], h[4 * q + 2] * sc[j], h[4 * q + 3] * sc[j])
                    : make_float4(h[4 * q], h[4 * q + 1], h[4 * q + 2], h[4 * q + 3]);
            if (a.s_self) {
                float ps = 0.f, pn = 0.f;
#pragma unroll
                for (int c = 0; c < F; ++c) { ps = fmaf(h[c], w_lds[F * F + c], ps); pn = fmaf(h[c], w_lds[F * F + F + c], pn); }
                a.s_self[row] = ps; a.s_neigh[row] = pn;
            }
        }
    }
}

struct SageArgs {
    const int32_t *rowptr; const int32_t *colidx; const float *X; int64_t ldx;
    const float *W; const float *bias; int C; float *Y; int64_t ldy; int self_loop; int n_rows;
};

template <int F>
__global__ __launch_bounds__(WAVES_PER_BLOCK * AMAR_WAVE) void sage_row_kernel(const SageArgs a) {
    constexpr int LPN = F / 4;
    const int lane = threadIdx.x & (AMAR_WAVE - 1);
    const int row = blockIdx.x * WAVES_PER_BLOCK + (threadIdx.x >> 6);
    if (row >= a.n_rows) return;
    const int q = lane % LPN, slot = lane / LPN;

    float wx[F], wa[F];
#pragma unroll
    for (int k = 0; k < F; ++k) {
        wx[k] = lane < a.C ? a.W[k * a.C + lane] : 0.f;
        wa[k] = lane < a.C ? a.W[(F + k) * a.C + lane] : 0.f;
    }
    const int beg = a.rowptr[row], end = a.rowptr[row + 1];
    float4 agg = row_gather_sum<LPN, false>(a.colidx, nullptr, a.X, a.ldx, beg, end, slot, q);
    const float4 xs = *reinterpret_cast<const float4 *>(a.X + (int64_t)row * a.ldx + 4 * q);
    float cnt = (float)(end - beg);
    if (a.self_loop) { agg = f4_add(agg, xs); cnt += 1.f; }
    cnt = fmaxf(cnt, 1.f);
    agg.x /= cnt; agg.y /= cnt; agg.z /= cnt; agg.w /= cnt;

    float fx[F], fa[F];
// ... 395 lines not shown
        if (F < 4 || (F & 3)) return AMAR_EUNSUPPORTED;
        for (int o = 0, w; o < F; o += w) {
            w = chunk_width(F - o);
            const int rc = amar_spmm_csr_f32(rowptr, colidx, vals, X + o, ldx, at(Y, o), ldy, n_rows, w, flags, at(bias, o),
                                             at(acc_in, o), ld_acc_in, at(acc_out, o), ld_acc_out, acc_div, stream);
            if (rc != AMAR_OK) return rc;
        }
        return AMAR_OK;
    }
    SpmmArgs a{};
    a.rowptr = rowptr; a.colidx = colidx; a.vals = vals; a.X = X; a.ldx = ldx; a.Y = Y; a.ldy = ldy;
    a.bias = (flags & AMAR_SPMM_BIAS) ? bias : nullptr; a.relu = (flags & AMAR_SPMM_RELU) ? 1 : 0;
    a.acc_in = acc_in; a.ld_acc_in = ld_acc_in; a.acc_out = acc_out; a.ld_acc_out = ld_acc_out;
    a.acc_div = acc_div; a.accum = accum ? 1 : 0; a.accum_div = (flags & AMAR_SPMM_ACCUM_DIV) ? 1 : 0;
    a.n_rows = n_rows;
    hipStream_t st = static_cast<hipStream_t>(stream);
    return vals ? launch_spmm<true, false>(a, F, st) : launch_spmm<false, false>(a, F, st);
}

int amar_gcn_layer_f32(const int32_t *rowptr, const int32_t *colidx, const float *vals,
                       const float *H, int64_t ldh, int32_t C, const float *bias,
                       float *Y, int64_t ldy,
                       const float *Wnext, int32_t Cn, float *Hnext, int64_t ldhn,
                       int32_t n_rows, amar_stream_t stream) {
    if (n_rows < 0 || !rowptr || !H || !Y || !bias) return AMAR_EINVAL;
    if (n_rows == 0) return AMAR_OK;
    if (!colidx) return AMAR_EINVAL;
    if (!ld_ok(ldh, C) || !ld_ok(ldy, C) || !amar_aligned16(H) || !amar_aligned16(Y) || !amar_aligned16(bias))
        return AMAR_EINVAL;
    if (Wnext && (!Hnext || Cn < 1 || ldhn < Cn)) return AMAR_EINVAL;
    if (Wnext && Cn > 64) return AMAR_EUNSUPPORTED;
    if (!native_width(C)) {
        if (C < 4 || (C & 3) || Wnext) return AMAR_EUNSUPPORTED;
        for (int o = 0, w; o < C; o += w) {
            w = chunk_width(C - o);
            const int rc = amar_gcn_layer_f32(rowptr, colidx, vals, H + o, ldh, w, bias + o, Y + o, ldy, nullptr, 0, nullptr, 0,
                                              n_rows, stream);
            if (rc != AMAR_OK) return rc;
        }
        return AMAR_OK;
    }
    SpmmArgs a{};
    a.rowptr = rowptr; a.colidx = colidx; a.vals = vals; a.X = H; a.ldx = ldh; a.Y = Y; a.ldy = ldy;
    a.bias = bias; a.relu = 1; a.Wn = Wnext; a.Cn = Cn; a.Hn = Hnext; a.ldhn = ldhn; a.n_rows = n_rows;
    hipStream_t st = static_cast<hipStream_t>(stream);
    if (Wnext) return vals ? launch_spmm<true, true>(a, C, st) : launch_spmm<false, true>(a, C, st);
    return vals ? launch_spmm<true, false>(a, C, st) : launch_spmm<false, false>(a, C, st);
}

static int rowwise_xw_run(const float *X, int64_t ldx, int32_t F, const float *W, int32_t C,
                          float *H, int64_t ldh, float *copy_to, int64_t ld_copy,
                          const float *a_self, const float *a_neigh, float *s_self, float *s_neigh,
                          const float *row_scale, const int32_t *row_ids, int32_t n_rows, amar_stream_t stream);

int amar_rowwise_xw_f32(const float *X, int64_t ldx, int32_t F, const float *W, int32_t C,
                        float *H, int64_t ldh, float *copy_to, int64_t ld_copy,
                        const float *a_self, const float *a_neigh, float *s_self, float *s_neigh,
                        const float *row_scale, int32_t n_rows, amar_stream_t stream) {
    return rowwise_xw_run(X, ldx, F, W, C, H, ldh, copy_to, ld_copy, a_self, a_neigh, s_self, s_neigh, row_scale, nullptr, n_rows, stream);
}

int amar_rowwise_xw_gather_f32(const float *X, int64_t ldx, int32_t F, const int32_t *row_ids, const float *W, int32_t C,
                               float *H, int64_t ldh, const float *row_scale, int32_t n_rows, amar_stream_t stream) {
    if (!row_ids) return AMAR_EINVAL;
    return rowwise_xw_run(X, ldx, F, W, C, H, ldh, nullptr, 0, nullptr, nullptr, nullptr, nullptr, row_scale, row_ids, n_rows, stream);
}

static int rowwise_xw_run(const float *X, int64_t ldx, int32_t F, const float *W, int32_t C,
                          float *H, int64_t ldh, float *copy_to, int64_t ld_copy,
                          const float *a_self, const float *a_neigh, float *s_self, float *s_neigh,
                          const float *row_scale, const int32_t *row_ids, int32_t n_rows, amar_stream_t stream) {
    if (n_rows < 0 || !X || !W || !H || F < 1 || C < 1 || ldx < F || ldh < C) return AMAR_EINVAL;
    if (F > 64 || C > 64) return AMAR_EUNSUPPORTED;
    if (copy_to && ld_copy < F) return AMAR_EINVAL;
    const bool attn = a_self || a_neigh || s_self || s_neigh;
    if (attn && !(a_self && a_neigh && s_self && s_neigh)) return AMAR_EINVAL;
    if (n_rows == 0) return AMAR_OK;
    int CP = 1;
    while (CP < C) CP <<= 1;
    if (attn && row_scale) return AMAR_EINVAL;
    XwArgs a{X, ldx, F, W, C, H, ldh, copy_to, ld_copy, a_self, a_neigh, attn ? s_self : nullptr, s_neigh, n_rows, row_scale, row_ids};
    if (F == C && (F == 8 || F == 16) && (ldx & 3) == 0 && (ldh & 3) == 0 && amar_aligned16(X) && amar_aligned16(H) &&
        (!copy_to || ((ld_copy & 3) == 0 && amar_aligned16(copy_to)))) {
        const int rows_per_block = F == 8 ? 512 : 256;
        int64_t vblocks = ((int64_t)n_rows + rows_per_block - 1) / rows_per_block;
        if (vblocks > 8192) vblocks = 8192;
        if (F == 8) hipLaunchKernelGGL(rowwise_xw_vec_kernel<8>, dim3((unsigned)vblocks), dim3(256), 0, static_cast<hipStream_t>(stream), a);
        else hipLaunchKernelGGL(rowwise_xw_vec_kernel<16>, dim3((unsigned)vblocks), dim3(256), 0, static_cast<hipStream_t>(stream), a);
        return amar_check_launch();
    }
    const int rows_per_block = 256 / CP;
    int64_t blocks = ((int64_t)n_rows + rows_per_block - 1) / rows_per_block;
    if (blocks > 8192) blocks = 8192;
    hipLaunchKernelGGL(rowwise_xw_kernel, dim3((unsigned)blocks), dim3(256), (size_t)F * C * sizeof(float),
                       static_cast<hipStream_t>(stream), a, CP);
    return amar_check_launch();
}

int amar_sage_layer_f32(const int32_t *rowptr, const int32_t *colidx,
                        const float *X, int64_t ldx, int32_t F,
                        const float *W, const float *bias, int32_t C,
                        float *Y, int64_t ldy, int32_t self_loop,
                        int32_t n_rows, amar_stream_t stream) {
    if (n_rows < 0 || !rowptr || !X || !W || !bias || !Y || C < 1 || ldy < C) return AMAR_EINVAL;
    if (!ld_ok(ldx, F) || !amar_aligned16(X)) return AMAR_EINVAL;
    if (C > 64) return AMAR_EUNSUPPORTED;
    if (n_rows == 0) return AMAR_OK;
    if (!colidx) return AMAR_EINVAL;
    SageArgs a{rowptr, colidx, X, ldx, W, bias, C, Y, ldy, self_loop ? 1 : 0, n_rows};
    const dim3 grid((n_rows + WAVES_PER_BLOCK - 1) / WAVES_PER_BLOCK), block(WAVES_PER_BLOCK * AMAR_WAVE);
    hipStream_t st = static_cast<hipStream_t>(stream);
    switch (F) {
    case 4:  hipLaunchKernelGGL(sage_row_kernel<4>, grid, block, 0, st, a); break;
    case 8:  hipLaunchKernelGGL(sage_row_kernel<8>, grid, block, 0, st, a); break;
    case 16: hipLaunchKernelGGL(sage_row_kernel<16>, grid, block, 0, st, a); break;
    case 32: hipLaunchKernelGGL(sage_row_kernel<32>, grid, block, 0, st, a); break;
    default: return AMAR_EUNSUPPORTED;
    }
    return amar_check_launch();
}

int amar_sage_tail_f32(const float *X, int64_t ldx, const float *AGG, int64_t lda, int32_t F,
                       const float *W, const float *bias, int32_t C, float *Y, int64_t ldy,
                       int64_t n_rows, amar_stream_t stream) {
    if (n_rows < 0 || !X || !AGG || !W || !bias || !Y || F < 4 || C < 4 || (F & 3) || (C & 3)) return AMAR_EINVAL;
    if (!ld_ok(ldx, F) || !ld_ok(lda, F) || !ld_ok(ldy, C) || !amar_aligned16(X) || !amar_aligned16(AGG) || !amar_aligned16(Y))
        return AMAR_EINVAL;
    if (F > 64 || C > 64) return AMAR_EUNSUPPORTED;
    if (n_rows == 0) return AMAR_OK;
    SageTailArgs a{X, ldx, AGG, lda, F, W, bias, C, Y, ldy, n_rows};
    const size_t lds = (size_t)(2 * F * C + C) * sizeof(float);
    int64_t blocks = (n_rows + 255) / 256;
    if (blocks > 8192) blocks = 8192;
    const dim3 grid((unsigned)blocks), block(256);
    hipStream_t st = static_cast<hipStream_t>(stream);
    if (C <= 4) hipLaunchKernelGGL(sage_tail_kernel<4>, grid, block, lds, st, a);
    else if (C <= 8) hipLaunchKernelGGL(sage_tail_kernel<8>, grid, block, lds, st, a);
    else if (C <= 16) hipLaunchKernelGGL(sage_tail_kernel<16>, grid, block, lds, st, a);
    else if (C <= 32) hipLaunchKernelGGL(sage_tail_kernel<32>, grid, block, lds, st, a);
    else hipLaunchKernelGGL(sage_tail_kernel<64>, grid, block, lds, st, a);
    return amar_check_launch();
}

static int gat_layer_launch(const int32_t *rowptr, const int32_t *colidx,
                            const float *H, int64_t ldh, int32_t C,
                            const float *s_self, const float *s_neigh, const float *bias,
                            float *Y, int64_t ldy, int32_t self_loop,
                            int32_t n_rows, const AmarDropout *drop, amar_stream_t stream) {
    if (n_rows < 0 || !rowptr || !H || !s_self || !s_neigh || !bias || !Y) return AMAR_EINVAL;
    if (!ld_ok(ldh, C) || !ld_ok(ldy, C) || !amar_aligned16(H) || !amar_aligned16(Y) || !amar_aligned16(bias))
        return AMAR_EINVAL;
    if (n_rows == 0) return AMAR_OK;
    if (!colidx) return AMAR_EINVAL;
    if (!native_width(C)) {
        if (C < 4 || (C & 3)) return AMAR_EUNSUPPORTED;
        for (int o = 0, w; o < C; o += w) {
            w = chunk_width(C - o);
            const int rc = gat_layer_launch(rowptr, colidx, H + o, ldh, w, s_self, s_neigh, bias + o, Y + o, ldy, self_loop,
                                            n_rows, drop, stream);
            if (rc != AMAR_OK) return rc;
        }
        return AMAR_OK;
    }
    GatArgs a{rowptr, colidx, H, ldh, s_self, s_neigh, bias, Y, ldy, self_loop ? 1 : 0, n_rows, drop ? *drop : AmarDropout{}};
    const dim3 grid((n_rows + WAVES_PER_BLOCK - 1) / WAVES_PER_BLOCK), block(WAVES_PER_BLOCK * AMAR_WAVE);
    hipStream_t st = static_cast<hipStream_t>(stream);
    if (drop) {
// ... 293 lines not shown
```

### deep_cbrs_amar_renaissance_amd/models/basic.py

```python
import abc

import os

import numpy as np

import torch

from deep_cbrs_amar_renaissance_amd import capi
from deep_cbrs_amar_renaissance_amd import recommend as rec
from deep_cbrs_amar_renaissance_amd.engine import Model, ids_to_device, to_device_tensor
from deep_cbrs_amar_renaissance_amd.models.dense import build_dense_network, build_dense_classifier
from deep_cbrs_amar_renaissance_amd.models.gnn import GCN, GAT, GraphSage, LightGCN, DGCF
from deep_cbrs_amar_renaissance_amd.models.tsgnn import TwoStepGCN, TwoStepGraphSage, TwoStepGAT, TwoStepLightGCN, TwoStepDGCF
from deep_cbrs_amar_renaissance_amd.models.twgnn import TwoWayGCN, TwoWayGraphSage, TwoWayGAT, TwoWayLightGCN, TwoWayDGCF


class BasicRS(Model):
    def __init__(
            self,
            dense_units=(512, 256, 128),
            clf_units=(64, 64),
            activation='relu',
            **kwargs
    ):
        super().__init__()
        self.dense_units = list(dense_units)
        self.unet = build_dense_network(dense_units, activation=activation)
        self.inet = build_dense_network(dense_units, activation=activation)
        self.clf = build_dense_classifier(clf_units, n_classes=1, activation=activation)

    def build(self, input_shape):
        self.build_head(input_shape[0][-1], input_shape[1][-1])

    def build_head(self, u_dim, i_dim):
        d = self.unet.build_chain(u_dim)
        self.inet.build_chain(i_dim)
        self.clf.build_chain(2 * d)
        self.built = True

    def call(self, inputs, u_ids=None, i_ids=None, **kwargs):
        u, i = inputs
        u, i = to_device_tensor(u), to_device_tensor(i)
        if len(self.dense_units) == 0:
            raise NotImplementedError("BasicRS needs at least one tower layer")
        if not self.built:
            self.build_head(u.shape[1], i.shape[1])
        towers = self.towers(u, i, u_ids=u_ids, i_ids=i_ids)
        return self.score_towers(towers, None, None)

    def fit(self, sequence, epochs=1, **kwargs):
        from deep_cbrs_amar_renaissance_amd import training
        return training.fit(self, sequence, epochs=epochs, **kwargs)

    def _split_plan(self, u_dim, i_dim):
        version = self.weights_version
        cache = getattr(self, '_split_cache', None)
        if cache is not None and cache[0] == (version, u_dim, i_dim):
            return cache[1]
        plan = None
        clf, d = list(self.clf.layers), self.dense_units[-1]
        if len(clf) >= 3:
            c1 = clf[0].units
            udims = [u_dim] + [l.units for l in self.unet.layers] + [c1]
            idims = [i_dim] + [l.units for l in self.inet.layers] + [c1]
            rdims = [c1] + [l.units for l in clf[1:]]
            if (capi.chain_supported(udims, u_dim) and capi.chain_supported(idims, i_dim)
                    and capi.chain_supported(rdims, c1, c1, sum_inputs=True)):
                w1 = clf[0].kernel.detach().cpu().numpy()
                b1 = clf[0].bias.detach().cpu().numpy()
                dev = clf[0].kernel.device
                np_ = lambda p: p.detach().cpu().numpy()
                ub, _ = capi.chain_pack([np_(l.kernel) for l in self.unet.layers] + [w1[:d]],
                                        [np_(l.bias) for l in self.unet.layers] + [0 * b1])
                ib, _ = capi.chain_pack([np_(l.kernel) for l in self.inet.layers] + [w1[d:]],
                                        [np_(l.bias) for l in self.inet.layers] + [b1])
                rb, _ = capi.chain_pack([np_(l.kernel) for l in clf[1:]], [np_(l.bias) for l in clf[1:]])
                to = lambda x: torch.from_numpy(x).to(dev)
                plan = {'u': (to(ub), udims, [l.activation for l in self.unet.layers] + [None]),
                        'i': (to(ib), idims, [l.activation for l in self.inet.layers] + [None]),
                        'rest': (to(rb), rdims, [l.activation for l in clf[1:]]), 'in_act': clf[0].activation}
        self._split_cache = ((version, u_dim, i_dim), plan)
        return plan

    def towers(self, u_table, i_table, u_ids=None, i_ids=None):
        plan = self._split_plan(u_table.shape[1], i_table.shape[1])
        if plan is None:
            return (self.unet.apply2(u_table, ids_a=u_ids), self.inet.apply2(i_table, ids_a=i_ids), False)
        out = []
        for key, table, ids in (('u', u_table, u_ids), ('i', i_table, i_ids)):
            blob, dims, acts = plan[key]
            m = ids.numel() if ids is not None else table.shape[0]
            t = torch.empty((m, dims[-1]), dtype=torch.float32, device=table.device)
            capi.chain(table, blob, dims, acts, t, ids_a=ids)
            out.append(t)
        return (out[0], out[1], True)

    def tower(self, key, table, ids=None):
        plan = self._split_plan(table.shape[1], table.shape[1])
        if plan is None:
            return (self.unet if key == 'u' else self.inet).apply2(table, ids_a=ids)
        blob, dims, acts = plan[key]
        m = ids.numel() if ids is not None else table.shape[0]
        t = torch.empty((m, dims[-1]), dtype=torch.float32, device=table.device)
        capi.chain(table, blob, dims, acts, t, ids_a=ids)
        return t

    def split_ready(self):
        return self._split_cache[1] is not None

    def score_towers(self, towers, u_ids, i_ids, u_base=0, i_base=0, pair_plan=None):
        tu, ti, split = towers
        if not split:
            return self.clf.apply2(tu, ti, ids_a=u_ids, base_a=u_base, ids_b=i_ids, base_b=i_base)
        plan = self._split_cache[1]
        blob, dims, acts = plan['rest']
        m = u_ids.numel() if u_ids is not None else tu.shape[0]
        out = torch.empty((m, 1), dtype=torch.float32, device=tu.device)
        if u_ids is None or i_ids is None:
            rows = getattr(self, '_row_ids', None)
            if rows is None or rows.numel() < m or rows.device != tu.device:
                rows = self._row_ids = torch.arange(max(m, 4096), dtype=torch.int32, device=tu.device)
            u_ids, u_base = (rows[:m], 0) if u_ids is None else (u_ids, u_base)
            i_ids, i_base = (rows[:m], 0) if i_ids is None else (i_ids, i_base)
        if pair_plan is not None:
            pair_plan.check(u_ids, i_ids)
            if pair_plan.mid_index is not None:
                capi.chain(tu, blob, dims, acts, pair_plan.mid.view(-1, 1), ids_a=pair_plan.u_ids, base_a=u_base, B=ti, ids_b=pair_plan.i_ids,
                           base_b=i_base, sum_inputs=True, in_act=plan['in_act'], out_index=pair_plan.mid_index)
                capi.scatter(pair_plan.mid, pair_plan.final_index, out, pair_plan.window_off, pair_plan.n_windows)
                return out
            capi.chain(tu, blob, dims, acts, out, ids_a=pair_plan.u_ids, base_a=u_base, B=ti, ids_b=pair_plan.i_ids, base_b=i_base,
                       sum_inputs=True, in_act=plan['in_act'], out_index=pair_plan.out_index)
            return out
        capi.chain(tu, blob, dims, acts, out, ids_a=u_ids, base_a=u_base, B=ti, ids_b=i_ids, base_b=i_base,
                   sum_inputs=True, in_act=plan['in_act'])
        return out

    def recommend(self, trainset, k=10, users=None, exclude_seen=True):
        rec.check_k(k)
        rec.check_users(users, len(trainset.users))
        tables = self._recommend_tables(trainset)
        split = self._recommend_split(*tables)
        if split is not None:
            return rec.fused(split, split[2], trainset, k, users, exclude_seen)
        return self._recommend_pairs(trainset, k, users, exclude_seen, towers=self.towers(*tables))

    def _recommend_pairs(self, trainset, k=10, users=None, exclude_seen=True, towers=None):
        rec.check_k(k)
        rec.check_users(users, len(trainset.users))
        towers = towers if towers is not None else self.towers(*self._recommend_tables(trainset))
        return rec.pairs(lambda u, i: self.score_towers(towers, u, i), trainset, k, users, exclude_seen, device=towers[0].device)

    def _recommend_route(self, trainset):
        d = np.asarray(trainset.embeddings).shape[1]
        if not self.built:
            self.build_head(d, d)
        return 'fused' if self._split_plan(d, d) is not None or self._rank_plan() is not None else 'pairs'

    def _recommend_tables(self, trainset):
        n_users, n_items = len(trainset.users), len(trainset.items)
        table = to_device_tensor(trainset.embeddings)
        if not self.built:
            self.build_head(table.shape[1], table.shape[1])
        return table[:n_users], table[n_users:n_users + n_items]

    def _rank_plan(self):
        clf = list(self.clf.layers)
        if len(clf) < 3 or clf[-1].units != 1 or len(clf) - 1 > capi.CHAIN_MAX_LAYERS + 1:
            return None
        rdims = [clf[0].units] + [l.units for l in clf[1:]]
        if max(rdims) > capi.CHAIN_MAX_WIDTH or rdims[0] % 4:
            return None
        np_ = lambda p: p.detach().cpu().numpy()
        rb, _ = capi.chain_pack([np_(l.kernel) for l in clf[1:]], [np_(l.bias) for l in clf[1:]])
        return {'rest': (torch.from_numpy(rb).to(clf[0].kernel.device), rdims, [l.activation for l in clf[1:]]), 'in_act': clf[0].activation}

    def _recommend_split(self, u_table, i_table):
        plan = self._split_plan(u_table.shape[1], i_table.shape[1])
        if plan is not None:
            tu, ti, _ = self.towers(u_table, i_table)
            return tu, ti, plan
        plan = self._rank_plan()
        if plan is None:
            return None
        tu_full, ti_full = self.unet.apply2(u_table), self.inet.apply2(i_table)
        l0 = self.clf.layers[0]
        w1, d, c1 = l0.kernel.detach(), tu_full.shape[1], l0.units
        tu = torch.empty((tu_full.shape[0], c1), dtype=torch.float32, device=tu_full.device)
        ti = torch.empty((ti_full.shape[0], c1), dtype=torch.float32, device=ti_full.device)
        capi.dense(tu_full, w1[:d].contiguous(), None, tu, act=None)
        capi.dense(ti_full, w1[d:].contiguous(), l0.bias.detach().contiguous(), ti, act=None)
        return tu, ti, plan

class PairPlan:

    N_XCD, CHUNK = 8, 128

    def __init__(self, u_ids, i_ids, phases=1):
        p = int(u_ids.numel())
        dev = u_ids.device
        pos = torch.arange(p, device=dev)
        per_phase = -(-p // phases)
        cls = (pos // per_phase) * self.N_XCD + (pos // self.CHUNK) % self.N_XCD
        n_cls = phases * self.N_XCD
        slots = torch.bincount(cls, minlength=n_cls)
        by_item = torch.argsort(i_ids.to(torch.int64), stable=True)
        order_cls = torch.arange(n_cls, device=dev).view(phases, self.N_XCD).t().reshape(-1)
        bucket_sizes = slots[order_cls]
        bucket_of_rank = torch.repeat_interleave(order_cls, bucket_sizes)
        order = by_item[torch.argsort((bucket_of_rank * (int(u_ids.max()) + 1) + u_ids[by_item].to(torch.int64)) * p + by_item)] if p else by_item
        place = torch.argsort(cls * p + pos)
        src = torch.empty(p, dtype=torch.int64, device=dev)
        src[place] = order
        self.u_ids = u_ids[src].contiguous()
        self.i_ids = i_ids[src].contiguous()
        self.out_index = src.to(torch.int32).contiguous()
        self._key = (u_ids.data_ptr(), i_ids.data_ptr(), p)
        self.window = 1 << max(16, min(19, int(round(np.log2(max(p, 1) / 185.0)))))
        self.mid_index = self.final_index = self.window_off = self.mid = None
        self.n_windows = 0
        if p > 2 * self.window and p >= int(os.environ.get('AMAR_PAIR_WINDOW_MIN', str(1 << 22))):
            n_win = -(-p // self.window)
            key = (src // self.window) * self.N_XCD + (pos // self.CHUNK) % self.N_XCD
            by_key = torch.argsort(key * p + pos)
            mid_index = torch.empty(p, dtype=torch.int32, device=dev)
            mid_index[by_key] = torch.arange(p, dtype=torch.int32, device=dev)
            self.mid_index = mid_index
            self.final_index = self.out_index[by_key].contiguous()
            counts = torch.bincount(src // self.window, minlength=n_win)
            self.window_off = torch.cat([torch.zeros(1, dtype=torch.int64, device=dev), torch.cumsum(counts, 0)]).to(torch.int32)
            self.n_windows = n_win
            self.mid = torch.empty(p, dtype=torch.float32, device=dev)

    def check(self, u_ids, i_ids):
        if (u_ids.data_ptr(), i_ids.data_ptr(), int(u_ids.numel())) != self._key:
            raise ValueError("this PairPlan was prepared for another pair list")


class BasicGNN(Model, abc.ABC):
    def __init__(
            self,
            dense_units=(32, 16),
            clf_units=(16, 16),
            activation='relu',
            **kwargs
    ):
        super().__init__()
        self.rs = BasicRS(dense_units, clf_units, activation=activation)
        self.n_users = self.n_items = None
        self._towers = None
        self.built = True

    def call(self, inputs, **kwargs):
        updated_embeddings = self.gnn(None)
        return self.embed_recommend(updated_embeddings, inputs)

    def embed_recommend(self, embeddings, inputs):
        n_nodes = embeddings.shape[0]
        u, i = ids_to_device(inputs[0], n_nodes), ids_to_device(inputs[1], n_nodes)
        if not self.gnn.hoist:
            return self.rs([embeddings, embeddings], u_ids=u, i_ids=i)
        key = (self.weights_version, embeddings.data_ptr())
        if self._towers is None or self._towers[0] != key:
            n = embeddings.shape[0]
            nu = self.n_users if self.n_users is not None else n
            lo = nu if self.n_users is not None else 0
            hi = nu + self.n_items if (self.n_users is not None and self.n_items is not None) else n
            self._towers = (key, self.rs.towers(embeddings[:nu], embeddings[lo:hi]), lo)
        _, towers, lo = self._towers
        return self.rs.score_towers(towers, u, i, 0, lo)

    def fit(self, sequence, epochs=1, **kwargs):
        from deep_cbrs_amar_renaissance_amd import training
        return training.fit(self, sequence, epochs=epochs, **kwargs)

    def recommend(self, trainset, k=10, users=None, exclude_seen=True):
        rec.check_k(k)
        rec.check_users(users, len(trainset.users))
        tables = self._recommend_tables(trainset)
        split = self.rs._recommend_split(*tables)
        if split is not None:
            return rec.fused(split, split[2], trainset, k, users, exclude_seen)
        return self._recommend_pairs(trainset, k, users, exclude_seen, towers=self.rs.towers(*tables))

    def _recommend_pairs(self, trainset, k=10, users=None, exclude_seen=True, towers=None):
        rec.check_k(k)
        rec.check_users(users, len(trainset.users))
        towers = towers if towers is not None else self.rs.towers(*self._recommend_tables(trainset))
        return rec.pairs(lambda u, i: self.rs.score_towers(towers, u, i), trainset, k, users, exclude_seen, device=towers[0].device)

    def _recommend_route(self, trainset):
        d = self.gnn.output_dim()
        return 'fused' if self.rs._split_plan(d, d) is not None or self.rs._rank_plan() is not None else 'pairs'

    def _recommend_tables(self, trainset):
        n_users, n_items = len(trainset.users), len(trainset.items)
        saved = (self.gnn.hoist, getattr(self.gnn, '_hoisted', None), self._towers)
        self.gnn.hoist = True
        try:
            emb = self.gnn(None)
        finally:
            self.gnn.hoist, self.gnn._hoisted, self._towers = saved
        return emb[:n_users], emb[n_users:n_users + n_items]

    def _hoist_begin(self, hoist):
        self.gnn.hoist = bool(hoist)
# ... 51 lines not shown
```

### deep_cbrs_amar_renaissance_amd/models/hybrid.py

```python
import abc
import os

import numpy as np
import torch

from deep_cbrs_amar_renaissance_amd import capi
from deep_cbrs_amar_renaissance_amd import recommend as rec
from deep_cbrs_amar_renaissance_amd.engine import Model, ids_to_device, to_device_tensor
from deep_cbrs_amar_renaissance_amd.layers.fusion import FusionLayer
from deep_cbrs_amar_renaissance_amd.models.dense import build_dense_classifier, build_dense_network, build_residual_dense_network
from deep_cbrs_amar_renaissance_amd.models.gnn import GCN, GAT, GraphSage, LightGCN, DGCF
from deep_cbrs_amar_renaissance_amd.models.tsgnn import TwoStepGCN, TwoStepGraphSage, TwoStepGAT, TwoStepLightGCN, TwoStepDGCF
from deep_cbrs_amar_renaissance_amd.models.twgnn import TwoWayGCN, TwoWayGraphSage, TwoWayGAT, TwoWayLightGCN, TwoWayDGCF


class HybridCBRS(Model):

    def __init__(
            self,
            feature_based=True,
            dense_units=((512, 256, 128), (512, 256, 128), (64, 64)),
            clf_units=(64, 64),
            activation='relu',
            fusion_method='concatenate',
# ... 105 lines not shown
        t3 = self.dense2b.apply2(ib_rows)
        if not self._can_fold():
            return t3
        d_first = self.dense2a.output_units if self.feature_based else self.dense1b.output_units
        _, wb, bias, _, _ = self._fold(None, None, self.dense3b, d_first)
        yb = torch.empty((t3.shape[0], wb.shape[1]), dtype=torch.float32, device=wb.device)
        capi.dense(t3, wb, bias, yb, act=None)
        return yb

    def _rest(self, net):
        key = ('rest', id(net), self.weights_version)
        cache = self.__dict__.setdefault('_rest_cache', {})
        if cache.get('key_' + str(id(net))) != key:
            layers = list(net.layers[1:])
            blob, dims = capi.chain_pack([l.kernel.detach().cpu().numpy() for l in layers],
                                         [l.bias.detach().cpu().numpy() for l in layers])
            cache['key_' + str(id(net))] = key
            cache[id(net)] = (torch.from_numpy(blob).to(layers[0].kernel.device), dims, [l.activation for l in layers],
                              net.layers[0].activation)
        return cache[id(net)]

    def _dual_plan(self):
        key = self.weights_version
        cache = self.__dict__.get('_dual_cache')
        if cache is not None and cache[0] == key:
            return cache[1]
        plan = None
        ra, rb, clf = list(self.dense3a.layers[1:]), list(self.dense3b.layers[1:]), list(self.clf.layers)
        D = self.dense3a.layers[0].units
        same = all(l.units == D for l in ra + rb) and self.dense3b.layers[0].units == D and len(ra) == len(rb) and \
            self.dense3a.layers[0].activation == self.dense3b.layers[0].activation and \
            all(x.activation == y.activation for x, y in zip(ra, rb))
        trunk_dims = [2 * D] + [l.units for l in clf]
        if capi.dual_chain_supported(D, same, trunk_dims):
            np_ = lambda prm: prm.detach().cpu().numpy()
            blobs = []
            for layers in (ra, rb, clf):
                if layers:
                    blob, _ = capi.chain_pack([np_(l.kernel) for l in layers], [np_(l.bias) for l in layers])
                    blobs.append(torch.from_numpy(blob))
            plan = {'D': D, 'in_act': self.dense3a.layers[0].activation, 'branch_acts': [l.activation for l in ra],
                    'trunk_dims': trunk_dims, 'trunk_acts': [l.activation for l in clf],
                    'wpack': torch.cat(blobs).to(clf[0].kernel.device)}
        self.__dict__['_dual_cache'] = (key, plan)
        return plan

    def score_towers(self, towers, u_ids, i_ids, u_base=0, i_base=0, pair_plan=None):
        tug, tig, tub, tib, folded = towers
        if self.feature_based:
            args1 = dict(ids_a=u_ids, base_a=u_base, ids_b=i_ids, base_b=i_base)
            args2 = args1
            in1, in2 = (tug, tig), (tub, tib)
        else:
            args1 = dict(ids_a=u_ids, base_a=u_base, ids_b=u_ids, base_b=u_base)
            args2 = dict(ids_a=i_ids, base_a=i_base, ids_b=i_ids, base_b=i_base)
            in1, in2 = (tug, tub), (tig, tib)
        plain = self.fuse2.method == 'concatenate' and self.residual is None
        if not folded:
            if self.fuse1a.method == 'concatenate':
                x1 = self.dense3a.apply2(in1[0], in1[1], **args1)
                x2 = self.dense3b.apply2(in2[0], in2[1], **args2)
            else:
                xs = []
                for fuse, net, (ta, tb), args in ((self.fuse1a, self.dense3a, in1, args1), (self.fuse1b, self.dense3b, in2, args2)):
                    ga, gb = self._rows(ta, args['ids_a'], args['base_a']), self._rows(tb, args['ids_b'], args['base_b'])
                    xs.append(net.apply2(fuse([ga, gb])))
                x1, x2 = xs
            return self.clf.apply2(x1, x2) if plain else self._tail(x1, x2)
        plan = self._dual_plan() if plain else None
        if plan is not None:
            m = args1['ids_a'].numel() if args1['ids_a'] is not None else in1[0].shape[0]
            out = torch.empty((m, 1), dtype=torch.float32, device=in1[0].device)
            if pair_plan is not None and u_ids is not None and i_ids is not None:
                pair_plan.check(u_ids, i_ids)
                pu, pi = pair_plan.u_ids, pair_plan.i_ids
                ia, ib = ((pu, pu), (pi, pi)) if self.feature_based else ((pu, pi), (pu, pi))
                two_step = pair_plan.mid_index is not None
                capi.dual_chain((in1[0], in2[0]), (in1[1], in2[1]), ia, ib,
                                (args1['base_a'], args2['base_a']), (args1['base_b'], args2['base_b']),
                                plan['D'], plan['in_act'], plan['branch_acts'], plan['trunk_dims'], plan['trunk_acts'], plan['wpack'],
                                pair_plan.mid.view(-1, 1) if two_step else out,
                                out_index=pair_plan.mid_index if two_step else pair_plan.out_index)
                if two_step:
                    capi.scatter(pair_plan.mid, pair_plan.final_index, out, pair_plan.window_off, pair_plan.n_windows)
                return out
            capi.dual_chain((in1[0], in2[0]), (in1[1], in2[1]), (args1['ids_a'], args2['ids_a']), (args1['ids_b'], args2['ids_b']),
                            (args1['base_a'], args2['base_a']), (args1['base_b'], args2['base_b']),
                            plan['D'], plan['in_act'], plan['branch_acts'], plan['trunk_dims'], plan['trunk_acts'], plan['wpack'], out)
            return out
        outs = []
        for net, (ta, tb), args in ((self.dense3a, in1, args1), (self.dense3b, in2, args2)):
            blob, dims, acts, in_act = self._rest(net)
            m = args['ids_a'].numel() if args['ids_a'] is not None else ta.shape[0]
            x = torch.empty((m, dims[-1]), dtype=torch.float32, device=ta.device)
            capi.chain(ta, blob, dims, acts, x, B=tb, sum_inputs=True, in_act=in_act, **args)
            outs.append(x)
        return self.clf.apply2(outs[0], outs[1]) if plain else self._tail(outs[0], outs[1])

    def recommend(self, trainset, k=10, users=None, exclude_seen=True):
        return self._recommend_pairs(trainset, k, users, exclude_seen)

    def _recommend_pairs(self, trainset, k=10, users=None, exclude_seen=True, towers=None):
        rec.check_k(k)
        rec.check_users(users, len(trainset.users))
        towers = towers if towers is not None else self._recommend_towers(trainset)
        return rec.pairs(lambda u, i: self.score_towers(towers, u, i), trainset, k, users, exclude_seen, device=towers[0].device)

    def _recommend_route(self, trainset):
        return 'pairs'

    def _recommend_towers(self, trainset):
        n_users, n_items = len(trainset.users), len(trainset.items)
        g, b = to_device_tensor(trainset.graph_embeddings), to_device_tensor(trainset.bert_embeddings)
        if not self.built:
            self.build_head(g.shape[1], b.shape[1])
        return self.towers(g[:n_users], g[n_users:n_users + n_items], b[:n_users], b[n_users:n_users + n_items])

    @staticmethod
    def _rows(table, ids, base):
        if ids is None:
            return table
        rows = torch.empty((ids.numel(), table.shape[1]), dtype=torch.float32, device=table.device)
        capi.copy_columns(table, rows, ids=ids, base=base)
        return rows

    def _tail(self, x1, x2):
        x = self.fuse2([x1, x2])
        if self.residual is None:
            return self.clf.apply2(x)
        r = self.residual.apply2(x)
        s = torch.empty_like(r)
        capi.add3_act(r, x1, x2, s, act=self.activation)
        return self.clf.apply2(s)


class HybridBertGNN(Model, abc.ABC):
    def __init__(
            self,
            dense_units=(32, 16),
            clf_units=(16, 16),
            feature_based=False,
            activation='relu',
            fusion_method='concatenate',
            residual=False,
            **kwargs
    ):
        super().__init__()
        self.rs = HybridCBRS(
            feature_based=feature_based,
            dense_units=dense_units,
            clf_units=clf_units,
            activation=activation,
            fusion_method=fusion_method,
            residual=residual
        )
        self.bert_table = None
        self.n_users = self.n_items = None
        self._towers = None
        self.built = True

    def set_bert_table(self, table):
        self.bert_table = to_device_tensor(table)

    def call(self, inputs, **kwargs):
        updated_embeddings = self.gnn(None)
        return self.embed_recommend(updated_embeddings, inputs)

# ... 126 lines not shown
```

### include/amar_hip.h

```cpp
#ifndef AMAR_HIP_H
#define AMAR_HIP_H

#include <stdint.h>

#ifdef __cplusplus
extern "C" {
#endif

#define AMAR_OK            0
#define AMAR_EINVAL       -1
#define AMAR_EUNSUPPORTED -2
#define AMAR_ELAUNCH      -3

#define AMAR_ACT_NONE     0
#define AMAR_ACT_RELU     1
#define AMAR_ACT_SIGMOID  2
#define AMAR_DENSE_WT 0x100

#define AMAR_SPMM_BIAS      1u
#define AMAR_SPMM_RELU      2u
#define AMAR_SPMM_ACCUM     4u
#define AMAR_SPMM_ACCUM_DIV 8u
#define AMAR_SPMM_SCALE_NEXT 16u
#define AMAR_SPMM_SAGE_TAIL 32u
// ... 39 lines not shown

int amar_rowwise_xw_f32(const float *X, int64_t ldx, int32_t F, const float *W, int32_t C,
                        float *H, int64_t ldh, float *copy_to, int64_t ld_copy,
                        const float *a_self, const float *a_neigh, float *s_self, float *s_neigh,
                        const float *row_scale, int32_t n_rows, amar_stream_t stream);

int amar_rowwise_xw_gather_f32(const float *X, int64_t ldx, int32_t F, const int32_t *row_ids, const float *W, int32_t C,
                               float *H, int64_t ldh, const float *row_scale, int32_t n_rows, amar_stream_t stream);

int amar_sage_layer_f32(const int32_t *rowptr, const int32_t *colidx,
                        const float *X, int64_t ldx, int32_t F,
                        const float *W, const float *bias, int32_t C,
                        float *Y, int64_t ldy, int32_t self_loop,
                        int32_t n_rows, amar_stream_t stream);

int amar_sage_tail_f32(const float *X, int64_t ldx, const float *AGG, int64_t lda, int32_t F,
                       const float *W, const float *bias, int32_t C, float *Y, int64_t ldy,
                       int64_t n_rows, amar_stream_t stream);

#define AMAR_AGG_SUM 0
#define AMAR_AGG_MAX 1
#define AMAR_AGG_MIN 2

int amar_sage_layer_agg_f32(const int32_t *rowptr, const int32_t *colidx,
                            const float *X, int64_t ldx, int32_t F,
                            const float *W, const float *bias, int32_t C,
                            float *Y, int64_t ldy, int32_t self_loop, int32_t op,
                            int32_t n_rows, amar_stream_t stream);

int amar_sage_aggregate_f32(const int32_t *rowptr, const int32_t *colidx,
                            const float *X, int64_t ldx, int32_t F,
                            float *AGG, int64_t lda, float *CNT, int64_t ldc,
                            int32_t self_loop, int32_t op, int32_t n_rows, amar_stream_t stream);

int amar_sage_aggregate_bwd_f32(const int32_t *rowptr, const int32_t *colidx,
                                const float *X, int64_t ldx, const float *AGG, int64_t lda,
                                const float *CNT, int64_t ldc, const float *DAGG, int64_t ldg, int32_t F,
                                float *pack, float *DX, int64_t lddx,
                                int32_t self_loop, int32_t n_rows, amar_stream_t stream);

int amar_gat_layer_f32(const int32_t *rowptr, const int32_t *colidx,
                       const float *H, int64_t ldh, int32_t C,
                       const float *s_self, const float *s_neigh, const float *bias,
                       float *Y, int64_t ldy, int32_t self_loop,
                       int32_t n_rows, amar_stream_t stream);

int amar_rowwise_xw_heads_f32(const float *X, int64_t ldx, int32_t F, const float *W, int32_t heads, int32_t C,
                              float *Hd, int64_t ldh, const float *a_self, const float *a_neigh, float *S,
                              int32_t n_rows, amar_stream_t stream);

int amar_gat_heads_f32(const int32_t *rowptr, const int32_t *colidx,
                       const float *Hd, int64_t ldh, int32_t heads, int32_t C,
                       const float *S, const float *bias, float *Y, int64_t ldy, float *out_tape,
                       int32_t concat, int32_t self_loop, int32_t n_rows, amar_stream_t stream);

int amar_dense_f32(const float *X, int64_t ldx, const int32_t *ids,
                   const float *W, const float *bias, float *Y, int64_t ldy,
                   int64_t M, int32_t K, int32_t N, int32_t act, amar_stream_t stream);

int64_t amar_dense_split_bytes(int32_t K, int32_t N);
int amar_dense_split_pack_f32(const float *W, int32_t K, int32_t N, void *out);
int amar_dense_split_f32(const float *X, int64_t ldx, const int32_t *ids, const void *Wq, const float *bias,
                         float *Y, int64_t ldy, int64_t M, int32_t K, int32_t N, int32_t act, amar_stream_t stream);

int64_t amar_chain_pack_floats(const int32_t *dims, int32_t n_layers);
int amar_chain_pack_f32(const float *const *kernels, const float *const *biases, const int32_t *dims,
                        int32_t n_layers, float *out);
int amar_chain_f32(const float *A, int64_t lda, int32_t Da, const int32_t *ids_a, int32_t base_a,
                   const float *B, int64_t ldb, int32_t Db, const int32_t *ids_b, int32_t base_b,
                   int32_t sum_inputs, int32_t in_act,
                   const float *wpack, const int32_t *dims, const int32_t *acts, int32_t n_layers,
                   float *out, int64_t ldo, int64_t P, amar_stream_t stream);

int amar_chain_indexed_f32(const float *A, int64_t lda, int32_t Da, const int32_t *ids_a, int32_t base_a,
                           const float *B, int64_t ldb, int32_t Db, const int32_t *ids_b, int32_t base_b,
                           int32_t sum_inputs, int32_t in_act,
                           const float *wpack, const int32_t *dims, const int32_t *acts, int32_t n_layers,
                           float *out, int64_t ldo, const int32_t *out_index, int64_t P, amar_stream_t stream);

int amar_chain_segments_f32(const float *const *seg, const int64_t *seg_ld, const int32_t *seg_width, int32_t n_seg,
                            const int32_t *ids, int32_t base,
                            const float *wpack, const int32_t *dims, const int32_t *acts, int32_t n_layers,
                            float *out, int64_t ldo, int64_t P, amar_stream_t stream);

#define AMAR_CHAIN_KERNEL_GENERIC 0
#define AMAR_CHAIN_KERNEL_PIPE 1
#define AMAR_CHAIN_KERNEL_ROWS 2
typedef struct amar_chain_route_info {
    int32_t kernel, maxt, full, am, split, scatter, shape, lastlin, seg, has_dot, layers, threads;
    int64_t blocks, lds_bytes;
} amar_chain_route_info;
int amar_chain_route(const float *A, int64_t lda, int32_t Da, const int32_t *ids_a, int32_t base_a,
                     const float *B, int64_t ldb, int32_t Db, const int32_t *ids_b, int32_t base_b,
                     int32_t sum_inputs, int32_t in_act,
                     const float *wpack, const int32_t *dims, const int32_t *acts, int32_t n_layers,
                     float *out, int64_t ldo, const int32_t *out_index, int64_t P, amar_chain_route_info *info);
int amar_chain_segments_route(const float *const *seg, const int64_t *seg_ld, const int32_t *seg_width, int32_t n_seg,
                              const int32_t *ids, int32_t base,
                              const float *wpack, const int32_t *dims, const int32_t *acts, int32_t n_layers,
                              float *out, int64_t ldo, int64_t P, amar_chain_route_info *info);

int amar_dual_chain_f32(const float *const *A, const int64_t *lda, const int32_t *const *ida, const int32_t *base_a,
                        const float *const *B, const int64_t *ldb, const int32_t *const *idb, const int32_t *base_b,
                        int32_t D, int32_t in_act, int32_t n_branch, const int32_t *branch_acts,
                        const int32_t *trunk_dims, const int32_t *trunk_acts, int32_t n_trunk,
                        const float *wpack, float *out, int64_t ldo, int64_t P, amar_stream_t stream);
int amar_dual_chain_indexed_f32(const float *const *A, const int64_t *lda, const int32_t *const *ida, const int32_t *base_a,
                                const float *const *B, const int64_t *ldb, const int32_t *const *idb, const int32_t *base_b,
                                int32_t D, int32_t in_act, int32_t n_branch, const int32_t *branch_acts,
                                const int32_t *trunk_dims, const int32_t *trunk_acts, int32_t n_trunk,
                                const float *wpack, float *out, int64_t ldo, const int32_t *out_index, int64_t P,
                                amar_stream_t stream);

int amar_copy_columns_f32(const float *src, int64_t lds, const int32_t *ids, int32_t base,
                          float *dst, int64_t ldd, int64_t n_rows, int32_t width, amar_stream_t stream);
int amar_reduce_layers_f32(const float *cat, int64_t ld, int32_t n_layers, int32_t width, float *out, int64_t ldo,
                           int64_t n_rows, int32_t mean, amar_stream_t stream);

int amar_scatter_f32(const float *src, const int32_t *index, float *dst, int64_t ldd, int64_t n,
                     const int32_t *window_off, int32_t n_windows, amar_stream_t stream);

int amar_reduce_layers_wsum_f32(const float *cat, int64_t ld, int32_t n_layers, int32_t width, const float *w, float *out, int64_t ldo,
                                int64_t n_rows, amar_stream_t stream);
int64_t amar_reduce_layers_wsum_bwd_scratch(void);
int amar_reduce_layers_wsum_bwd_f32(const float *cat, int64_t ld, int32_t n_layers, int32_t width, const float *w,
                                    const float *d_out, int64_t ldd, float *d_cat, int64_t ld_dcat, float *dw, float *scratch,
                                    int64_t n_rows, amar_stream_t stream);

int amar_gat_xs_f32(const int32_t *rowptr, const int32_t *colidx, int32_t n_slices,
                    const float *H, int64_t ldh, int32_t C, const float *s_self, const float *s_neigh, const float *bias,
                    float *packed, float *partials, float *Y, int64_t ldy, int32_t self_loop, int32_t n_rows,
                    int32_t n_cols, int32_t row_offset, amar_stream_t stream);

int amar_gat_lt_f32(const int32_t *words, const int32_t *stream_start, const int32_t *wsteps, const int32_t *tile_row0,
                    const int32_t *n_win, const int32_t *vstart, const int32_t *vcount, int32_t n_tiles, int32_t maxwin1, int32_t pace_every,
                    int32_t rows_per_wave, const float *diag, const int32_t *rowptr, const int32_t *colidx,
                    const float *H, int64_t ldh, int32_t C, const float *s_self, const float *s_neigh, const float *s_neigh_max,
                    const float *bias, float *Y, int64_t ldy, int32_t self_loop, int32_t n_rows, int32_t n_cols, int32_t row_offset,
                    amar_stream_t stream);
int amar_gat_lt_rows_per_wave(int32_t C);
int amar_colmax_f32(const float *x, int64_t n, float *out, amar_stream_t stream);

int amar_attention_mix_f32(const float *A, int64_t lda, const float *B, int64_t ldb, const float *TA, int64_t ldta,
                           const float *TB, int64_t ldtb, float *out, int64_t ldo, int64_t M, int32_t D, amar_stream_t stream);
int amar_attention_mix_bwd_f32(const float *dOut, int64_t ldd, const float *A, int64_t lda, const float *B, int64_t ldb,
                               const float *TA, int64_t ldta, const float *TB, int64_t ldtb,
                               float *dA, float *dB, float *dTA, float *dTB, int64_t M, int32_t D, amar_stream_t stream);
int amar_add3_act_f32(const float *A, int64_t lda, const float *B, int64_t ldb, const float *C, int64_t ldc, float *out, int64_t ldo,
                      int64_t M, int32_t W, int32_t act, amar_stream_t stream);
int amar_locality_scale_f32(const float *X, int64_t ldx, const float *w, float *out, int64_t ldo, int64_t M, int32_t W,
                            amar_stream_t stream);
int amar_locality_scale_bwd_f32(const float *dOut, int64_t ldd, const float *X, int64_t ldx, const float *w, float *dX, int64_t lddx,
                                float *dw, int64_t M, int32_t W, int32_t accumulate, amar_stream_t stream);

int amar_act_bwd_f32(const float *dY, int64_t ldd, const float *Y, int64_t ldy, float *dZ, int64_t ldz,
                     int64_t M, int32_t N, int32_t act, amar_stream_t stream);
int64_t amar_wgrad_scratch_floats(int64_t M, int32_t K, int32_t N);
int amar_dense_stack_f32(const float *X, int64_t ldx, const int32_t *ids, float *Xcopy, int64_t ldxc, int32_t n_layers,
                         const float *const *W, const float *const *bias, const int32_t *dims, const int32_t *acts,
                         float *const *Y, const int64_t *ldy, int64_t M, amar_stream_t stream);
typedef struct amar_dense_stack_desc {
    const float *X; int64_t ldx; const int32_t *ids; float *Xcopy; int64_t ldxc; int32_t n_layers;
    const float *const *W; const float *const *bias; const int32_t *dims; const int32_t *acts; float *const *Y; const int64_t *ldy; int64_t M;
} amar_dense_stack_desc;
int amar_dense_stack_pair_f32(const amar_dense_stack_desc *s0, const amar_dense_stack_desc *s1, amar_stream_t stream);
typedef struct amar_dense_stack_route_info {
    int32_t rows, vec_x, vec_w[4];
    int64_t groups, lds_bytes;
} amar_dense_stack_route_info;
int amar_dense_stack_route(const float *X, int64_t ldx, const int32_t *ids, float *Xcopy, int64_t ldxc, int32_t n_layers,
                           const float *const *W, const float *const *bias, const int32_t *dims, const int32_t *acts,
                           float *const *Y, const int64_t *ldy, int64_t M, amar_dense_stack_route_info *out);
int64_t amar_dense_stack_bwd_groups(int64_t M);
int64_t amar_dense_stack_bwd_workspace_floats(int64_t M, int32_t n_layers, const int32_t *dims);
int amar_dense_stack_bwd_f32(const float *dYtop, int64_t lddy, const float *Ytop, int64_t ldytop, int32_t n_layers,
                             const float *const *X, const int64_t *ldx, const float *const *W, const int32_t *dims, const int32_t *acts,
                             float *dX0, int64_t lddx0, float *const *dW, float *const *db, float *workspace, int32_t flags,
                             int64_t M, amar_stream_t stream);
typedef struct amar_dense_stack_bwd_desc {
    const float *dYtop; int64_t lddy; const float *Ytop; int64_t ldytop; int32_t n_layers;
    const float *const *X; const int64_t *ldx; const float *const *W; const int32_t *dims; const int32_t *acts;
    float *dX0; int64_t lddx0; float *const *dW; float *const *db; float *workspace; int32_t flags; int64_t M;
} amar_dense_stack_bwd_desc;
int amar_dense_stack_bwd_pair_f32(const amar_dense_stack_bwd_desc *s0, const amar_dense_stack_bwd_desc *s1, amar_stream_t stream);
typedef struct amar_dense_stack_bwd_route_info {
    int32_t rows, vec_top, vec_x[4], vec_w[4];
    int64_t groups, lds_bytes;
} amar_dense_stack_bwd_route_info;
int amar_dense_stack_bwd_route(const float *dYtop, int64_t lddy, const float *Ytop, int64_t ldytop, int32_t n_layers,
                               const float *const *X, const int64_t *ldx, const float *const *W, const int32_t *dims, const int32_t *acts,
                               float *dX0, int64_t lddx0, float *const *dW, float *const *db, float *workspace, int32_t flags,
                               int64_t M, amar_dense_stack_bwd_route_info *out);
#define AMAR_DENSE_BWD_DEFER 0x100
#define AMAR_DENSE_BWD_ACCUM_DX 0x200
int64_t amar_dense_bwd_groups(int64_t M);
int64_t amar_dense_bwd_workspace_floats(int64_t M, int32_t K, int32_t N);
#define AMAR_DENSE_BWD_KERNEL_TILE 0
#define AMAR_DENSE_BWD_KERNEL_ROWS 1
typedef struct amar_dense_bwd_route_info {
    int32_t kernel, mt, kp, np, vec, x_scalar, subtiles, fold, fold_launch;
    int64_t launched_groups, out_groups;
} amar_dense_bwd_route_info;
int amar_dense_bwd_route(const float *X, int64_t ldx, const float *Y, int64_t ldy, const float *dY, int64_t lddy, const float *W, int32_t act,
// ... 148 lines not shown
```

Before: 11.92 billion pairs/s.

## Fuse user/item towers into one launch, add LDS windowed scatter, retune XW rows

The user and item tower MLPs now run in a single chain_rows launch, with the grid split between the two inputs. The separate launches are kept as a fallback when shapes differ. A new scatter kernel places pair scores into an LDS image per output window of 40960 entries, then writes each window back contiguously. The pair plan's sort key now also orders by dispatch round. The F=8 row-wise XW kernel processes 4 rows per thread instead of 2. Together these aim to cut launch count, make the final scatter's writes coalesced, and improve locality, at the cost of larger LDS use and a more complex index ordering.

```diff
diff --git a/deep_cbrs_amar_renaissance_amd/capi.py b/deep_cbrs_amar_renaissance_amd/capi.py
--- a/deep_cbrs_amar_renaissance_amd/capi.py
+++ b/deep_cbrs_amar_renaissance_amd/capi.py
@@ -51,6 +51,7 @@
     'amar_chain_pack_f32': (ctypes.c_int, [_P, _P, _P, _I32, _P]),
     'amar_chain_f32': (ctypes.c_int, [_P, _I64, _I32, _P, _I32, _P, _I64, _I32, _P, _I32, _I32, _I32, _P, _P, _P, _I32, _P, _I64, _I64, _P]),
     'amar_chain_indexed_f32': (ctypes.c_int, [_P, _I64, _I32, _P, _I32, _P, _I64, _I32, _P, _I32, _I32, _I32, _P, _P, _P, _I32, _P, _I64, _P, _I64, _P]),
+    'amar_chain_pair_f32': (ctypes.c_int, [_P, _P, _I32, _P, _P, _P, _P, _P, _I32, _P, _P, _P, _P]),
     'amar_chain_segments_f32': (ctypes.c_int, [_P, _P, _P, _I32, _P, _I32, _P, _P, _P, _I32, _P, _I64, _I64, _P]),
     'amar_chain_route': (ctypes.c_int, [_P, _I64, _I32, _P, _I32, _P, _I64, _I32, _P, _I32, _I32, _I32, _P, _P, _P, _I32, _P, _I64, _P, _I64, _P]),
     'amar_chain_segments_route': (ctypes.c_int, [_P, _P, _P, _I32, _P, _I32, _P, _P, _P, _I32, _P, _I64, _I64, _P]),
@@ -58,6 +59,7 @@
     'amar_dual_chain_indexed_f32': (ctypes.c_int, [_P, _P, _P, _P, _P, _P, _P, _P, _I32, _I32, _I32, _P, _P, _P, _I32, _P, _P, _I64, _P, _I64, _P]),
     'amar_copy_columns_f32': (ctypes.c_int, [_P, _I64, _P, _I32, _P, _I64, _I64, _I32, _P]),
     'amar_scatter_f32': (ctypes.c_int, [_P, _P, _P, _I64, _I64, _P, _I32, _P]),
+    'amar_scatter_windows_f32': (ctypes.c_int, [_P, _P, _P, _I64, _I64, _I32, _P]),
     'amar_reduce_layers_f32': (ctypes.c_int, [_P, _I64, _I32, _I32, _P, _I64, _I64, _I32, _P]),
     'amar_reduce_layers_wsum_f32': (ctypes.c_int, [_P, _I64, _I32, _I32, _P, _P, _I64, _I64, _P]),
     'amar_reduce_layers_wsum_bwd_scratch': (ctypes.c_int64, []),
@@ -789,6 +791,25 @@
     _check(load().amar_chain_indexed_f32(*args, _stream()), 'amar_chain_indexed_f32' if out_index is not None else 'amar_chain_f32')
 
 
+def chain_pair(tables, wpacks, dims, acts, outs, ids=(None, None), bases=(0, 0)):
+    for t, o, i in zip(tables, outs, ids):
+        if (i is not None and i.numel() != o.shape[0]) or (i is None and t.shape[0] < o.shape[0]) or t.shape[1] != dims[0]:
+            raise ValueError("chain_pair: one input row (or id) of dims[0] features per output row expected")
+    arr = lambda vals, ctype: (ctype * 2)(*vals)
+    ld = lambda t, nm: _ld(t, nm) if t.shape[0] else max(int(t.shape[1]), 1)
+    code = load().amar_chain_pair_f32(
+        arr([_ptr_entries(t, torch.float32, 'A') for t in tables], ctypes.c_void_p), arr([ld(t, 'A') for t in tables], ctypes.c_int64), int(dims[0]),
+        arr([_ptr_entries(i, torch.int32, 'ids') for i in ids], ctypes.c_void_p), arr([int(b) for b in bases], ctypes.c_int32),
+        arr([_ptr(w, torch.float32, 'wpack') for w in wpacks], ctypes.c_void_p), (ctypes.c_int32 * len(dims))(*dims),
+        (ctypes.c_int32 * len(acts))(*[ACT_CODES[a] for a in acts]), len(acts),
+        arr([_ptr_entries(o, torch.float32, 'out') for o in outs], ctypes.c_void_p), arr([ld(o, 'out') for o in outs], ctypes.c_int64),
+        arr([int(o.shape[0]) for o in outs], ctypes.c_int64), _stream())
+    if code == -2:
+        return False
+    _check(code, 'amar_chain_pair_f32')
+    return True
+
+
 CHAIN_KERNEL_GENERIC, CHAIN_KERNEL_PIPE, CHAIN_KERNEL_ROWS = 0, 1, 2
 
 
@@ -855,11 +876,25 @@
     _check(code, 'amar_dual_chain_f32' if out_index is None else 'amar_dual_chain_indexed_f32')
 
 
-def scatter(src, index, dst, window_off=None, n_windows=1):
+def scatter_windows(src, index, dst, window):
+    n = int(index.numel())
+    if src.numel() < n:
+        raise ValueError("scatter_windows: one source value per index expected")
+    code = load().amar_scatter_windows_f32(_ptr(src, torch.float32, 'src'), _ptr(index, torch.int32, 'index'), _ptr(dst, torch.float32, 'dst'),
+                                           _ld(dst, 'dst') if dst.dim() == 2 else 1, n, int(window), _stream())
+    if code == -2:
+        return False
+    _check(code, 'amar_scatter_windows_f32')
+    return True
+
+
+def scatter(src, index, dst, window_off=None, n_windows=1, window=None):
     n = int(index.numel())
     if src.numel() < n or (window_off is not None and window_off.numel() != n_windows + 1):
         raise ValueError("scatter: one source value per index and n_windows + 1 window offsets expected")
     if n == 0:
+        return
+    if window is not None and scatter_windows(src, index, dst, window):
         return
     _check(load().amar_scatter_f32(_ptr(src, torch.float32, 'src'), _ptr(index, torch.int32, 'index'), _ptr(dst, torch.float32, 'dst'),
                                    _ld(dst, 'dst') if dst.dim() == 2 else 1, n, _ptr(window_off, torch.int32, 'window_off'),
diff --git a/deep_cbrs_amar_renaissance_amd/csrc/amar_chain.hip b/deep_cbrs_amar_renaissance_amd/csrc/amar_chain.hip
--- a/deep_cbrs_amar_renaissance_amd/csrc/amar_chain.hip
+++ b/deep_cbrs_amar_renaissance_amd/csrc/amar_chain.hip
@@ -22,6 +22,7 @@
     int n_out;
     float *out; int64_t ldo; int64_t P;
     const int32_t *out_index;
+    int blocks2; const float *A2; int64_t lda2; const int32_t *ids_a2; int base_a2; const float *wpack2; float *out2; int64_t ldo2; int64_t P2;
 };
 
 __device__ __forceinline__ int64_t chain_out_row(const ChainArgs &a, int64_t p) { return a.out_index ? (int64_t)a.out_index[p] : p; }
@@ -171,18 +172,26 @@
 __global__ __launch_bounds__(256) void chain_rows_kernel(const ChainArgs a) {
     constexpr int NL = shape_nl(SHAPE), T0 = shape_t(SHAPE, 0), TN = shape_t(SHAPE, NL), MAXT = shape_maxt(SHAPE);
     extern __shared__ __attribute__((aligned(16))) float w_lds[];
+    const uint32_t blocks1 = gridDim.x - (uint32_t)a.blocks2;
+    const bool second = !SEG && blockIdx.x >= blocks1;
+    const float *const A_ = second ? a.A2 : a.A, *const wpack = second ? a.wpack2 : a.wpack;
+    const int32_t *const ids = second ? a.ids_a2 : a.ids_a;
+    const int base_a = second ? a.base_a2 : a.base_a;
+    float *const out = second ? a.out2 : a.out;
+    const int64_t ldo = second ? a.ldo2 : a.ldo;
+    const uint32_t bid = second ? blockIdx.x - blocks1 : blockIdx.x, nblk = second ? (uint32_t)a.blocks2 : blocks1;
     for (int i = threadIdx.x * 4; i < a.wpack_floats; i += blockDim.x * 4)
-        *reinterpret_cast<float4 *>(&w_lds[i]) = *reinterpret_cast<const float4 *>(a.wpack + i);
+        *reinterpret_cast<float4 *>(&w_lds[i]) = *reinterpret_cast<const float4 *>(wpack + i);
     __syncthreads();
 
     const int lane = threadIdx.x & 63, g = lane >> 4, col = lane & 15;
     constexpr uint32_t rows_per_wave = 16 * PT;
-    const uint32_t stride = gridDim.x * 4 * rows_per_wave;
-    const uint32_t P = (uint32_t)a.P, last = P - 1;
-    const uint32_t lda = (uint32_t)a.lda * 4u;
+    const uint32_t stride = nblk * 4 * rows_per_wave;
+    const uint32_t P = (uint32_t)(second ? a.P2 : a.P), last = P - 1;
+    const uint32_t lda = (uint32_t)(second ? a.lda2 : a.lda) * 4u;
     const int f_last = 16 * (T0 - 1) + 4 * g;
     const bool tail_ok = f_last < a.Da;
-    const char *Ag = reinterpret_cast<const char *>(a.A) + 16 * g;
+    const char *Ag = reinterpret_cast<const char *>(A_) + 16 * g;
     const int tail_off = tail_ok ? 64 * (T0 - 1) : -16 * g;
     const char *seg_base[SEG ? T0 : 1];
     uint32_t seg_ldb[SEG ? T0 : 1];
@@ -202,7 +211,7 @@
 #pragma unroll
         for (int pt = 0; pt < PT; ++pt) {
             const uint32_t p = min(b + 16 * pt + col, last);
-            const uint32_t row = a.ids_a ? (uint32_t)(a.ids_a[p] - a.base_a) : p;
+            const uint32_t row = ids ? (uint32_t)(ids[p] - base_a) : p;
             const char *pa = Ag + (uint64_t)row * lda;
 #pragma unroll
             for (int t = 0; t < T0; ++t) {
@@ -212,7 +221,7 @@
         }
     };
 
-    uint32_t base = (blockIdx.x * 4 + (threadIdx.x >> 6)) * rows_per_wave;
+    uint32_t base = (bid * 4 + (threadIdx.x >> 6)) * rows_per_wave;
     if (base >= P) return;
     gather(base);
     for (; base < P; base += stride) {
@@ -258,7 +267,7 @@
 #pragma unroll
         for (int pt = 0; pt < PT; ++pt) {
             const uint32_t p = base + 16 * pt + col;
-            float *po = a.out + (int64_t)p * a.ldo + 4 * g;
+            float *po = out + (int64_t)p * ldo + 4 * g;
 #pragma unroll
             for (int m = 0; m < TN; ++m)
                 if (p < P && 16 * m + 4 * g < a.n_out) *reinterpret_cast<f32x4 *>(po + 16 * m) = x[m][pt];
@@ -1132,6 +1141,25 @@
     ChainArgs a;
     return chain_route(seg[0], seg_ld[0], (int32_t)da, ids, base, nullptr, 0, 0, nullptr, 0, 0, AMAR_ACT_NONE, wpack, dims, acts, n_layers, out, ldo,
                        nullptr, P, n_seg, seg, seg_ld, seg_width, a, *info);
+}
+
+static int chain_rows_launch(const ChainArgs &a, const amar_chain_route_info &r, dim3 grid, hipStream_t st) {
+    const dim3 block((unsigned)r.threads);
+    const size_t lds = (size_t)r.lds_bytes;
+#define AMAR_ROWS_CASE(NLL, A0, A1, A2, A3)                                                                                      \
+        case chain_shape(NLL, A0, A1, A2, A3):                                                                                   \
+            if (r.seg) {                                                                                                         \
+                if (r.lastlin) hipLaunchKernelGGL((chain_rows_kernel<chain_shape(NLL, A0, A1, A2, A3), 2, true, true>), grid, block, lds, st, a);   \
+                else hipLaunchKernelGGL((chain_rows_kernel<chain_shape(NLL, A0, A1, A2, A3), 2, false, true>), grid, block, lds, st, a);            \
+            } else if (r.lastlin) hipLaunchKernelGGL((chain_rows_kernel<chain_shape(NLL, A0, A1, A2, A3), 2, true, false>), grid, block, lds, st, a);   \
+            else hipLaunchKernelGGL((chain_rows_kernel<chain_shape(NLL, A0, A1, A2, A3), 2, false, false>), grid, block, lds, st, a);            \
+            break;
+    switch (r.shape) {
+    AMAR_ROWS_SHAPES(AMAR_ROWS_CASE)
+    default: return AMAR_EUNSUPPORTED;
+    }
+#undef AMAR_ROWS_CASE
+    return amar_check_launch();
 }
 
 static int chain_run(const float *A, int64_t lda, int32_t Da, const int32_t *ids_a, int32_t base_a,
@@ -1163,22 +1191,7 @@
 #undef AMAR_PIPE_LAUNCH
         return amar_check_launch();
     }
-    if (r.kernel == AMAR_CHAIN_KERNEL_ROWS) {
-#define AMAR_ROWS_CASE(NLL, A0, A1, A2, A3)                                                                                      \
-        case chain_shape(NLL, A0, A1, A2, A3):                                                                                   \
-            if (r.seg) {                                                                                                         \
-                if (r.lastlin) hipLaunchKernelGGL((chain_rows_kernel<chain_shape(NLL, A0, A1, A2, A3), 2, true, true>), grid, block, lds, st, a);   \
-                else hipLaunchKernelGGL((chain_rows_kernel<chain_shape(NLL, A0, A1, A2, A3), 2, false, true>), grid, block, lds, st, a);            \
-            } else if (r.lastlin) hipLaunchKernelGGL((chain_rows_kernel<chain_shape(NLL, A0, A1, A2, A3), 2, true, false>), grid, block, lds, st, a);   \
-            else hipLaunchKernelGGL((chain_rows_kernel<chain_shape(NLL, A0, A1, A2, A3), 2, false, false>), grid, block, lds, st, a);            \
-            break;
-        switch (r.shape) {
-        AMAR_ROWS_SHAPES(AMAR_ROWS_CASE)
-        default: return AMAR_EUNSUPPORTED;
-        }
-#undef AMAR_ROWS_CASE
-        return amar_check_launch();
-    }
+    if (r.kernel == AMAR_CHAIN_KERNEL_ROWS) return chain_rows_launch(a, r, grid, st);
 #define AMAR_CHAIN_LAUNCH(MT)                                                                                           \
     do {                                                                                                                \
         auto kern = r.full ? (r.am == 1 ? chain_kernel<MT, 2, true, 1> : r.am == 2 ? chain_kernel<MT, 2, true, 2>       \
@@ -1194,6 +1207,25 @@
     if (r.maxt == 3) AMAR_CHAIN_LAUNCH(3); else if (r.maxt == 4) AMAR_CHAIN_LAUNCH(4); else AMAR_CHAIN_LAUNCH(8);
 #undef AMAR_CHAIN_LAUNCH
     return amar_check_launch();
+}
+
+int amar_chain_pair_f32(const float *const *A, const int64_t *lda, int32_t Da, const int32_t *const *ids, const int32_t *base,
+                        const float *const *wpack, const int32_t *dims, const int32_t *acts, int32_t n_layers,
+                        float *const *out, const int64_t *ldo, const int64_t *P, amar_stream_t stream) {
+    if (!A || !lda || !ids || !base || !wpack || !out || !ldo || !P) return AMAR_EINVAL;
+    ChainArgs a[2];
+    amar_chain_route_info r[2];
+    for (int s = 0; s < 2; ++s)
+        if (const int rc = chain_route(A[s], lda[s], Da, ids[s], base[s], nullptr, 0, 0, nullptr, 0, 0, AMAR_ACT_NONE, wpack[s], dims, acts,
+                                       n_layers, out[s], ldo[s], nullptr, P[s], 0, nullptr, nullptr, nullptr, a[s], r[s]))
+            return rc;
+    if (r[0].kernel != AMAR_CHAIN_KERNEL_ROWS || r[1].kernel != AMAR_CHAIN_KERNEL_ROWS) return AMAR_EUNSUPPORTED;
+    if (r[0].blocks + r[1].blocks == 0) return AMAR_OK;
+    ChainArgs &m = a[0];
+    m.blocks2 = (int)r[1].blocks;
+    m.A2 = a[1].A; m.lda2 = a[1].lda; m.ids_a2 = a[1].ids_a; m.base_a2 = a[1].base_a; m.wpack2 = a[1].wpack;
+    m.out2 = a[1].out; m.ldo2 = a[1].ldo; m.P2 = a[1].P;
+    return chain_rows_launch(m, r[0], dim3((unsigned)(r[0].blocks + r[1].blocks)), static_cast<hipStream_t>(stream));
 }
 
 int amar_dual_chain_f32(const float *const *A, const int64_t *lda, const int32_t *const *ida, const int32_t *base_a,
diff --git a/deep_cbrs_amar_renaissance_amd/csrc/amar_layout.hip b/deep_cbrs_amar_renaissance_amd/csrc/amar_layout.hip
--- a/deep_cbrs_amar_renaissance_amd/csrc/amar_layout.hip
+++ b/deep_cbrs_amar_renaissance_amd/csrc/amar_layout.hip
@@ -119,6 +119,53 @@
     }
 }
 
+constexpr int SW_THREADS = 1024, SW_UNROLL = 8, SW_MAX_WINDOW = 160 * 1024 / 4;
+
+__device__ __forceinline__ void sw_place(float *img, int32_t index, int32_t lo, uint32_t count, float v) {
+    const uint32_t rel = (uint32_t)index - (uint32_t)lo;
+    if (rel < count) img[rel] = v;
+}
+
+__global__ __launch_bounds__(SW_THREADS) void scatter_windows_lds_kernel(const float *__restrict__ src, const int32_t *__restrict__ index,
+                                                                         float *__restrict__ dst, int32_t n, int32_t window, int32_t n_windows) {
+    extern __shared__ __attribute__((aligned(16))) float img[];
+    for (int w = blockIdx.x; w < n_windows; w += gridDim.x) {
+        const int32_t lo = w * window;
+        const uint32_t count = (uint32_t)min(window, n - lo);
+        const int quads = (int)(count >> 2);
+        const float4 *s4 = reinterpret_cast<const float4 *>(src + lo);
+        const int4 *i4 = reinterpret_cast<const int4 *>(index + lo);
+        int q = threadIdx.x;
+        for (; q + (SW_UNROLL - 1) * SW_THREADS < quads; q += SW_UNROLL * SW_THREADS) {
+            int4 ix[SW_UNROLL];
+            float4 v[SW_UNROLL];
+#pragma unroll
+            for (int u = 0; u < SW_UNROLL; ++u) ix[u] = i4[q + u * SW_THREADS];
+#pragma unroll
+            for (int u = 0; u < SW_UNROLL; ++u) v[u] = s4[q + u * SW_THREADS];
+#pragma unroll
+            for (int u = 0; u < SW_UNROLL; ++u) {
+                sw_place(img, ix[u].x, lo, count, v[u].x); sw_place(img, ix[u].y, lo, count, v[u].y);
+                sw_place(img, ix[u].z, lo, count, v[u].z); sw_place(img, ix[u].w, lo, count, v[u].w);
+            }
+        }
+        for (; q < quads; q += SW_THREADS) {
+            const int4 ix = i4[q];
+            const float4 v = s4[q];
+            sw_place(img, ix.x, lo, count, v.x); sw_place(img, ix.y, lo, count, v.y);
+            sw_place(img, ix.z, lo, count, v.z); sw_place(img, ix.w, lo, count, v.w);
+        }
+        const uint32_t t = 4u * quads + threadIdx.x;
+        if (t < count) sw_place(img, index[lo + t], lo, count, src[lo + t]);
+        __syncthreads();
+        float4 *d4 = reinterpret_cast<float4 *>(dst + lo);
+        const float4 *m4 = reinterpret_cast<const float4 *>(img);
+        for (q = threadIdx.x; q < quads; q += SW_THREADS) d4[q] = m4[q];
+        if (t < count) dst[lo + t] = img[t];
+        __syncthreads();
+    }
+}
+
 }
 
 extern "C" {
@@ -186,4 +233,29 @@
                        window_off, n_windows, per_xcd);
     return amar_check_launch();
 }
-}
+
+int amar_scatter_windows_f32(const float *src, const int32_t *index, float *dst, int64_t ldd, int64_t n, int32_t window,
+                             amar_stream_t stream) {
+    if (n < 0 || !src || !index || !dst || ldd < 1 || window < 1) return AMAR_EINVAL;
+    if (ldd != 1 || window > SW_MAX_WINDOW || n >= (1ll << 31)) return AMAR_EUNSUPPORTED;
+    if ((window & 3) || !amar_aligned16(src) || !amar_aligned16(index) || !amar_aligned16(dst)) return AMAR_EUNSUPPORTED;
+    if (n == 0) return AMAR_OK;
+    const int64_t n_windows = (n + window - 1) / window;
+    const size_t lds_bytes = (size_t)(((n < window ? n : window) + 3) & ~3ll) * sizeof(float);
+    static bool lds_ok[AMAR_MAX_DEVICES];
+    if (lds_bytes > 64 * 1024)
+        if (const int rc = amar_allow_lds(reinterpret_cast<const void *>(scatter_windows_lds_kernel), SW_MAX_WINDOW * sizeof(float), lds_ok)) return rc;
+    static int cus[AMAR_MAX_DEVICES];
+    int dev = 0;
+    if (hipGetDevice(&dev) != hipSuccess || dev < 0 || dev >= AMAR_MAX_DEVICES) return AMAR_ELAUNCH;
+    if (!cus[dev] && (hipDeviceGetAttribute(&cus[dev], hipDeviceAttributeMultiprocessorCount, dev) != hipSuccess || cus[dev] < 1)) {
+        cus[dev] = 0;
+        return AMAR_ELAUNCH;
+    }
+    const int64_t slots = cus[dev] >= 8 ? cus[dev] & ~7 : cus[dev];
+    const unsigned blocks = (unsigned)(n_windows < slots ? n_windows : slots);
+    hipLaunchKernelGGL(scatter_windows_lds_kernel, dim3(blocks), dim3(SW_THREADS), lds_bytes, static_cast<hipStream_t>(stream), src, index, dst,
+                       (int32_t)n, window, (int32_t)n_windows);
+    return amar_check_launch();
+}
+}
diff --git a/deep_cbrs_amar_renaissance_amd/csrc/amar_propagate.hip b/deep_cbrs_amar_renaissance_amd/csrc/amar_propagate.hip
--- a/deep_cbrs_amar_renaissance_amd/csrc/amar_propagate.hip
+++ b/deep_cbrs_amar_renaissance_amd/csrc/amar_propagate.hip
@@ -974,7 +974,7 @@
     for (int i = threadIdx.x; i < F * F; i += 256) w_lds[i] = a.W[i];
     if (a.s_self) for (int i = threadIdx.x; i < F; i += 256) { w_lds[F * F + i] = a.a_self[i]; w_lds[F * F + F + i] = a.a_neigh[i]; }
     __syncthreads();
-    constexpr int R = F == 8 ? 2 : 1;
+    constexpr int R = F == 8 ? 4 : 1;
     for (int64_t row0 = (int64_t)blockIdx.x * 256 * R + threadIdx.x; row0 < a.n_rows; row0 += (int64_t)gridDim.x * 256 * R) {
         float x[R][F], sc[R];
         bool pad[R];
@@ -1536,7 +1536,7 @@
     XwArgs a{X, ldx, F, W, C, H, ldh, copy_to, ld_copy, a_self, a_neigh, attn ? s_self : nullptr, s_neigh, n_rows, row_scale, row_ids};
     if (F == C && (F == 8 || F == 16) && (ldx & 3) == 0 && (ldh & 3) == 0 && amar_aligned16(X) && amar_aligned16(H) &&
         (!copy_to || ((ld_copy & 3) == 0 && amar_aligned16(copy_to)))) {
-        const int rows_per_block = F == 8 ? 512 : 256;
+        const int rows_per_block = F == 8 ? 1024 : 256;
         int64_t vblocks = ((int64_t)n_rows + rows_per_block - 1) / rows_per_block;
         if (vblocks > 8192) vblocks = 8192;
         if (F == 8) hipLaunchKernelGGL(rowwise_xw_vec_kernel<8>, dim3((unsigned)vblocks), dim3(256), 0, static_cast<hipStream_t>(stream), a);
diff --git a/deep_cbrs_amar_renaissance_amd/models/basic.py b/deep_cbrs_amar_renaissance_amd/models/basic.py
--- a/deep_cbrs_amar_renaissance_amd/models/basic.py
+++ b/deep_cbrs_amar_renaissance_amd/models/basic.py
@@ -88,11 +88,13 @@
             return (self.unet.apply2(u_table, ids_a=u_ids), self.inet.apply2(i_table, ids_a=i_ids), False)
         out = []
         for key, table, ids in (('u', u_table, u_ids), ('i', i_table, i_ids)):
-            blob, dims, acts = plan[key]
             m = ids.numel() if ids is not None else table.shape[0]
-            t = torch.empty((m, dims[-1]), dtype=torch.float32, device=table.device)
-            capi.chain(table, blob, dims, acts, t, ids_a=ids)
-            out.append(t)
+            out.append(torch.empty((m, plan[key][1][-1]), dtype=torch.float32, device=table.device))
+        (ub, udims, uacts), (ib, idims, iacts) = plan['u'], plan['i']
+        if not (udims == idims and uacts == iacts and isinstance(u_table, torch.Tensor) and isinstance(i_table, torch.Tensor)
+                and capi.chain_pair((u_table, i_table), (ub, ib), udims, uacts, out, ids=(u_ids, i_ids))):
+            capi.chain(u_table, ub, udims, uacts, out[0], ids_a=u_ids)
+            capi.chain(i_table, ib, idims, iacts, out[1], ids_a=i_ids)
         return (out[0], out[1], True)
 
     def tower(self, key, table, ids=None):
@@ -127,7 +129,7 @@
             if pair_plan.mid_index is not None:
                 capi.chain(tu, blob, dims, acts, pair_plan.mid.view(-1, 1), ids_a=pair_plan.u_ids, base_a=u_base, B=ti, ids_b=pair_plan.i_ids,
                            base_b=i_base, sum_inputs=True, in_act=plan['in_act'], out_index=pair_plan.mid_index)
-                capi.scatter(pair_plan.mid, pair_plan.final_index, out, pair_plan.window_off, pair_plan.n_windows)
+                capi.scatter(pair_plan.mid, pair_plan.final_index, out, pair_plan.window_off, pair_plan.n_windows, window=pair_plan.window)
                 return out
             capi.chain(tu, blob, dims, acts, out, ids_a=pair_plan.u_ids, base_a=u_base, B=ti, ids_b=pair_plan.i_ids, base_b=i_base,
                        sum_inputs=True, in_act=plan['in_act'], out_index=pair_plan.out_index)
@@ -195,6 +197,8 @@
 class PairPlan:
 
     N_XCD, CHUNK = 8, 128
+    LDS_WINDOW, LDS_WINDOW_MAX_PAIRS = 40960, 1 << 26
+    GRID, ROUNDS = 1536, 3
 
     def __init__(self, u_ids, i_ids, phases=1):
         p = int(u_ids.numel())
@@ -217,11 +221,14 @@
         self.out_index = src.to(torch.int32).contiguous()
         self._key = (u_ids.data_ptr(), i_ids.data_ptr(), p)
         self.window = 1 << max(16, min(19, int(round(np.log2(max(p, 1) / 185.0)))))
+        if p <= self.LDS_WINDOW_MAX_PAIRS:
+            self.window = self.LDS_WINDOW
         self.mid_index = self.final_index = self.window_off = self.mid = None
         self.n_windows = 0
         if p > 2 * self.window and p >= int(os.environ.get('AMAR_PAIR_WINDOW_MIN', str(1 << 22))):
             n_win = -(-p // self.window)
-            key = (src // self.window) * self.N_XCD + (pos // self.CHUNK) % self.N_XCD
+            rnd = ((pos // self.CHUNK) % self.GRID) * self.ROUNDS // self.GRID
+            key = ((src // self.window) * self.N_XCD + (pos // self.CHUNK) % self.N_XCD) * self.ROUNDS + rnd
             by_key = torch.argsort(key * p + pos)
             mid_index = torch.empty(p, dtype=torch.int32, device=dev)
             mid_index[by_key] = torch.arange(p, dtype=torch.int32, device=dev)
diff --git a/deep_cbrs_amar_renaissance_amd/models/hybrid.py b/deep_cbrs_amar_renaissance_amd/models/hybrid.py
--- a/deep_cbrs_amar_renaissance_amd/models/hybrid.py
+++ b/deep_cbrs_amar_renaissance_amd/models/hybrid.py
@@ -211,7 +211,7 @@
                                 pair_plan.mid.view(-1, 1) if two_step else out,
                                 out_index=pair_plan.mid_index if two_step else pair_plan.out_index)
                 if two_step:
-                    capi.scatter(pair_plan.mid, pair_plan.final_index, out, pair_plan.window_off, pair_plan.n_windows)
+                    capi.scatter(pair_plan.mid, pair_plan.final_index, out, pair_plan.window_off, pair_plan.n_windows, window=pair_plan.window)
                 return out
             capi.dual_chain((in1[0], in2[0]), (in1[1], in2[1]), (args1['ids_a'], args2['ids_a']), (args1['ids_b'], args2['ids_b']),
                             (args1['base_a'], args2['base_a']), (args1['base_b'], args2['base_b']),
diff --git a/include/amar_hip.h b/include/amar_hip.h
--- a/include/amar_hip.h
+++ b/include/amar_hip.h
@@ -145,6 +145,10 @@
                             const int32_t *ids, int32_t base,
                             const float *wpack, const int32_t *dims, const int32_t *acts, int32_t n_layers,
                             float *out, int64_t ldo, int64_t P, amar_stream_t stream);
+
+int amar_chain_pair_f32(const float *const *A, const int64_t *lda, int32_t Da, const int32_t *const *ids, const int32_t *base,
+                        const float *const *wpack, const int32_t *dims, const int32_t *acts, int32_t n_layers,
+                        float *const *out, const int64_t *ldo, const int64_t *P, amar_stream_t stream);
 
 #define AMAR_CHAIN_KERNEL_GENERIC 0
 #define AMAR_CHAIN_KERNEL_PIPE 1
@@ -182,6 +186,9 @@
 
 int amar_scatter_f32(const float *src, const int32_t *index, float *dst, int64_t ldd, int64_t n,
                      const int32_t *window_off, int32_t n_windows, amar_stream_t stream);
+
+int amar_scatter_windows_f32(const float *src, const int32_t *index, float *dst, int64_t ldd, int64_t n, int32_t window,
+                             amar_stream_t stream);
 
 int amar_reduce_layers_wsum_f32(const float *cat, int64_t ld, int32_t n_layers, int32_t width, const float *w, float *out, int64_t ldo,
                                 int64_t n_rows, amar_stream_t stream);
```

Measured after the change: 12.39 billion pairs/s (median of 6 runs). 1.04x the previous value.
